# Blaizzy/mlx-audio

Hardware: NVIDIA H100
Metric: audio-sec/sec Kokoro-82M TTS (128-phoneme utterance, 9.75 s) (higher is better)
Workload: dtype bf16x2

## Files before the change

### include/b200audio.h

```cpp
#ifndef B200AUDIO_H
#define B200AUDIO_H

#include <stdint.h>

#ifdef __cplusplus
extern "C" {
#endif

#define B2A_OK 0
#define B2A_E_INVALID (-1)
#define B2A_E_CUDA (-2)
#define B2A_E_UNSUPPORTED (-3)

enum {
  B2A_ACT_NONE = 0,
  B2A_ACT_LRELU = 1,
  B2A_ACT_SNAKE = 2,
  B2A_ACT_ELU = 3,
  B2A_ACT_GELU = 4,
  B2A_ACT_GELU_TANH = 5,
  B2A_ACT_TANH = 6,
  B2A_ACT_SIGMOID = 7,
  B2A_ACT_SILU = 8,
  B2A_ACT_CLIP1 = 9
};

const char* b2a_last_error(void);
int32_t b2a_version(void);
int32_t b2a_device_sm_count(void);

typedef struct {
  const float* x; int64_t x_bs; int64_t x_ld;
  int32_t B, L, Cin;
  const float* w; const float* bias;
  float* y; int64_t y_bs; int64_t y_ld;
  int32_t Lout, Cout;
  int32_t K, stride, dilation, pad_left, groups, pad_mode;
  const float* pre_scale; const float* pre_shift;
  int32_t pre_act; float pre_p0; const float* pre_a; const float* pre_b;
  int32_t post_act; float post_p0;
  const float* post_cscale; int64_t post_cscale_bs;
  const float* res; int64_t res_bs; int64_t res_ld; int32_t res_div;
  float out_scale; int32_t accumulate;
  void* emit_hi; void* emit_lo; int64_t emit_ld;
  int32_t emit_act; float emit_p0; const float* emit_a; const float* emit_b;
} b2a_conv1d_t;

int32_t b2a_conv1d_cl(const b2a_conv1d_t* p, void* stream);
int32_t b2a_convtr1d_cl(const b2a_conv1d_t* p, void* stream);

enum {
  B2A_CONV_PATH_LINEAR_ROWS = 1,
  B2A_CONV_PATH_NARROW = 2,
  B2A_CONV_PATH_DENSE = 3,
  B2A_CONV_PATH_DW_TILED4 = 4,
  B2A_CONV_PATH_DW_TILED = 5,
  B2A_CONV_PATH_DW = 6,
  B2A_CONV_PATH_CONVTR_DENSE = 7,
  B2A_CONV_PATH_CONVTR_DW = 8
};
int32_t b2a_conv1d_cl_last_path(int32_t* out4);

int32_t b2a_kokoro_source_conv(const float* x, int32_t B, int32_t L, const float* w, const float* bias, float* y, int32_t Lout,
                               int32_t Cout, int32_t K, int32_t stride, int32_t pad_left, void* stream);

int32_t b2a_prep_bf16(const float* x, int64_t x_bs, int64_t x_ld, int32_t B, int32_t L, int32_t C, int32_t cpad,
                      const float* scale, const float* shift, int32_t act, float p0, const float* a, const float* b,
                      void* hi, void* lo, int32_t f16, void* stream);
int32_t b2a_conv1d_tc(const void* a_hi, const void* a_lo, int32_t f16, int32_t B, int32_t L, int32_t cin_pad, const void* w_bf16,
                      const void* w_lo,
                      int32_t taps, const int32_t* shifts_host, int32_t Cout, int32_t Lout, const float* bias,
                      int32_t post_act, float post_p0, const float* cscale, int64_t cscale_bs, const float* res,
                      int64_t res_bs, int64_t res_ld, int32_t res_div, float out_scale, int32_t accumulate, float* y,
                      int64_t y_bs, int64_t y_ld, int32_t up_stride, int32_t up_crop, void* emit_hi, void* emit_lo,
                      int64_t emit_ld, void* attn_ws, int32_t attn_heads, float attn_scale, void* stream);

typedef struct {
  int32_t T, layers, heads, hidden, inter, planes;
  const void* w[4];
  const float* bias[4];
  const float* ln_w[2];
  const float* ln_b[2];
  float eps, scale;
  float* h; void* h_hi; void* h_lo;
} b2a_albert_t;
int64_t b2a_albert_ws_bytes(int32_t T, int32_t heads, int32_t hidden, int32_t inter);
int32_t b2a_albert_encoder(const b2a_albert_t* a, void* ws, uint32_t* err, int64_t* timeline, void* stream);

int32_t b2a_conv1d_tc_debug(void* dbg8);

int32_t b2a_conv1d_tc_last_config(int32_t* out5);

int32_t b2a_copy2d(const float* src, int64_t src_ld, float* dst, int64_t dst_ld, int64_t rows, int32_t cols, void* stream);
int32_t b2a_gather_rows(const float* src, int64_t src_ld, const int64_t* idx, float* dst, int64_t dst_ld,
                        int64_t rows, int32_t cols, int64_t n_src_rows, const float* add, int64_t add_ld, int64_t add_period,
                        void* stream);
int32_t b2a_durations_to_index(const float* dur_f, const int64_t* dur_i, int32_t T, float speed, int64_t* pred_dur_out,
                               int64_t* idx_out, int64_t max_frames, int64_t* total_dev, void* stream);

int64_t b2a_adain_ws_bytes(int32_t B, int32_t L, int32_t C);
int32_t b2a_adain_coeffs(const float* x, int64_t x_bs, int64_t x_ld, int32_t B, int32_t L, int32_t C,
                         const float* gb, float eps, float* scale, float* shift, void* ws, void* stream);
int32_t b2a_channel_stats(const float* x, int64_t x_bs, int64_t x_ld, int32_t B, int32_t L, int32_t C, int64_t* const* dst,
                          const int64_t* dst_bs, int32_t n_dst, void* stream);
int32_t b2a_coeffs_from_stats(const int64_t* stats, int32_t B, int32_t L, int32_t C, const float* gb, float eps, float* scale, float* shift,
                              void* stream);
int32_t b2a_layernorm(const float* x, int64_t x_ld, const float* res, int64_t res_ld, float* y, int64_t y_ld,
                      int64_t rows, int32_t C, const float* w, const float* b, const float* ada, float eps,
                      int32_t rms, int32_t post_act, float post_p0, void* emit_hi, void* emit_lo, int64_t emit_ld, void* stream);

typedef struct {
  const float* q; const float* k; const float* v; float* o;
  int64_t q_bs, q_ld, k_bs, k_ld, v_bs, v_ld, o_bs, o_ld;
  int32_t B, Tq, Tk, H, Hkv, D;
  float scale; int32_t causal, q_offset, window;
  const int32_t* k_len;
  void* emit_hi; void* emit_lo; int64_t emit_ld;
  int32_t operands_ready;
} b2a_attn_t;
int32_t b2a_attention(const b2a_attn_t* p, void* stream);
int64_t b2a_attention_tc_ws_bytes(int32_t B, int32_t H, int32_t Tq, int32_t Tk);
int32_t b2a_attention_tc(const b2a_attn_t* p, void* ws, void* stream);
int32_t b2a_rope(float* x, int64_t x_bs, int64_t x_ld, int32_t B, int32_t T, int32_t H, int32_t D,
                 int32_t offset, float base, int32_t traditional, void* stream);

int32_t b2a_lstm_bidir(const float* xproj, const float* wh, float* out, int64_t out_ld, int32_t B, int32_t T, int32_t H, void* stream);

int32_t b2a_stft(const float* x, int64_t x_bs, int32_t B, int64_t n, const float* window, int32_t n_fft, int32_t hop,
                 int32_t pad_mode, int64_t frames, float* out_re, float* out_im, void* stream);
int32_t b2a_whisper_logmel(const float* x, int64_t x_bs, int32_t B, int64_t n, int64_t padding, const float* window,
                           const float* filters, int32_t n_mels, int64_t frames, float* out, float* gmax, void* stream);
int32_t b2a_istft(const float* re, const float* im, int32_t B, int32_t n_fft, int32_t T, int32_t hop, const float* window,
                  int32_t norm_sq, int32_t clamp_mode, int64_t trim, int64_t out_len, float* out, float* ws, void* stream);

int32_t b2a_resample_poly(const float* x, int64_t x_bs, int32_t B, int64_t n_in, const double* h, int32_t n_h, int32_t up,
                          int32_t down, int64_t n_pre_pad, int64_t n_pre_remove, float* out, int64_t n_out, void* stream);

int32_t b2a_kokoro_source(const float* f0, int32_t B, int32_t n_frames, int32_t n_down, const float* noise, const float* lin_w,
                          const float* lin_b, float* har, float* src_ws, double* ph_ws, void* stream);
int32_t b2a_kokoro_istft_head(const float* x, int64_t x_bs, int64_t x_ld, int32_t B, int32_t T, float* audio, void* stream);

#define B2A_CONVF_MAX_PROBLEMS 4
typedef struct {
  const float* x; const float* x1; const float* x2; int64_t x_bs, x_ld; float in_scale;
  int32_t B, L, Cin;
  int32_t pre_mode; const float* pre_scale; const float* pre_shift; const int64_t* pre_stats; const float* pre_gb; int64_t pre_gb_bs; float pre_eps;
  int32_t pre_act; float pre_p0; const float* pre_a; const float* pre_b;
  const void* w_hi; const void* w_lo; int32_t cin_pad, taps, N; int32_t shifts[32];
  int32_t Lout; const float* bias; int32_t post_act; float post_p0; const float* cscale; int64_t cscale_bs;
  const float* res; int64_t res_bs, res_ld; int32_t res_div; float out_scale; int32_t accumulate;
  float* y; int64_t y_bs, y_ld;
  int32_t up_stride, up_crop;
  int64_t* stats_out;
} b2a_convf_t;
int32_t b2a_conv1d_fused_debug(void* stamps );
int32_t b2a_conv1d_fused(const b2a_convf_t* problems, int32_t n_problems, int32_t planes, int32_t f16, void* ws, int64_t ws_bytes, void* stream);
int32_t b2a_conv1d_fused_fits(int32_t span, int32_t N, int32_t C, int32_t wplanes, int32_t planes);
int32_t b2a_conv1d_fused_last_config(int32_t* out10);

int32_t b2a_randn(float* out, int64_t n, uint64_t seed, uint64_t offset, void* stream);
int32_t b2a_randn_dev(float* out, int64_t n, uint64_t* state, void* stream);

int32_t b2a_whisper_greedy_step(const float* logits, int64_t logits_bs, const int64_t* tokens, int64_t tokens_bs,
                                int32_t B, int32_t cur_len, int32_t sample_begin, int32_t V, const float* suppress_mask,
                                const float* blank_mask, int32_t eot, int32_t no_timestamps, int32_t timestamp_begin,
                                int32_t max_initial_ts, int32_t without_timestamps, int64_t* next_out,
                                float* sum_logprobs, int32_t* not_done, float temperature, const float* u, void* stream);

int32_t b2a_sample_token(const float* logits, int64_t logits_bs, int32_t B, int32_t V, const float* suppress_mask,
                         uint8_t* seen, int64_t seen_bs, int32_t mark_seen, float repetition_penalty, float temperature,
                         int32_t top_k, float top_p, float min_p, const float* u, int64_t* out, int64_t out_stride,
                         float* filtered_out, uint8_t* finished, int32_t eos, void* stream);

int32_t b2a_gemv_bf16(const float* x, int64_t x_ld, int32_t M, int32_t K, const void* w_bf16, int64_t w_ld, int32_t N,
                      const float* bias, const float* norm_w, float norm_eps, int32_t mode, const float* res, int64_t res_ld,
                      float* y, int64_t y_ld, const void* prefetch, int64_t prefetch_bytes, void* stream);
int32_t b2a_qknorm_rope_cache(const float* qkv, int64_t qkv_bs, int64_t qkv_ss, int32_t B, int32_t S, int32_t Hq, int32_t Hkv,
                              int32_t D, const float* q_norm_w, const float* k_norm_w, float eps, const int32_t* pos3,
                              const int32_t* base_dev, int32_t base_host, int32_t sec_h, int32_t sec_w, float theta,
                              float* q_out, int64_t qo_bs, int64_t qo_ss, float* k_cache, float* v_cache, int64_t c_bs,
                              int64_t c_ss, int32_t smax, const int32_t* pos_shift, const int32_t* base_rows, const int32_t* slot,
                              void* stream);
int32_t b2a_attn_decode(const float* q, int64_t q_bs, int64_t q_ss, const float* k_cache, const float* v_cache, int64_t c_bs,
                        int64_t c_ss, float* out, int64_t o_bs, int64_t o_ss, int32_t B, int32_t S, int32_t Hq, int32_t Hkv,
                        int32_t D, float scale, const int32_t* base_dev, int32_t base_host, const int32_t* kv_start,
                        int32_t max_k, const int32_t* base_rows, const int32_t* slot, void* stream);
int32_t b2a_attn_prefill(const float* q, int64_t q_bs, int64_t q_ss, const float* k_cache, const float* v_cache, int64_t c_bs,
                         int64_t c_ss, float* out, int64_t o_bs, int64_t o_ss, int32_t B, int32_t S, int32_t Hq, int32_t Hkv,
                         int32_t D, float scale, const int32_t* base_dev, int32_t base_host, const int32_t* kv_start,
                         int32_t max_k, const int32_t* base_rows, const int32_t* slot, void* stream);
int32_t b2a_swiglu(const float* x, int64_t x_ld, int64_t rows, int32_t I, int32_t interleaved, float* y, int64_t y_ld, void* stream);
int32_t b2a_embed_sum(const int64_t* codes, int64_t codes_bs, int32_t B, int32_t G, int32_t dim, const float* const* tables_dev,
                      const int32_t* bins_dev, const float* text, int64_t text_bs, int64_t text_ss, int32_t n_text,
                      const float* pad, const int32_t* step_dev, int32_t step_sub, float* out, int64_t out_bs,
                      int32_t* err_flag_dev, int32_t* tidx, const uint8_t* finished, void* stream);
int32_t b2a_incr_i32(int32_t* p, int32_t v, void* stream);
int32_t b2a_slot_advance(int32_t* lengths, int32_t* frames, uint8_t* finished, const int32_t* cap, const int64_t* codes, int32_t G,
                         int64_t* out, int64_t out_bs, const float* u_tab, int64_t u_bs, float* u, int32_t B, void* stream);

int32_t b2a_rvq_decode(const int64_t* codes, int64_t codes_bs, int64_t codes_qs, int32_t B, int32_t nq, int64_t T,
                       const float* codebooks, int32_t bins, int32_t dim, float* out, int64_t out_ld, int32_t* err_flag_dev, void* stream);
int32_t b2a_rvq_encode(const float* x, int64_t x_ld, int64_t rows, int32_t dim, const float* codebooks, const double* c2, int32_t bins,
                       int32_t nq, int32_t mode, int64_t* codes, int64_t codes_row_stride, int64_t codes_level_stride, void* stream);
int32_t b2a_snac_from_codes(const int64_t* const* codes_host_ptrs, const int32_t* strides_host, int32_t n_levels,
                            const float* const* emb_host_ptrs, const float* const* w_host_ptrs, const float* const* bias_host_ptrs,
                            int32_t B, int64_t T, int32_t bins, int32_t cd, int32_t dim, float* out, int32_t* err_flag_dev, void* stream);

typedef struct {
  const float* w_in; const float* b_in;
  const float* cbn; const double* c2;
  const float* cb;
  const float* w_out; const float* b_out;
  int32_t cd; int32_t lat_off;
} b2a_dac_level_t;
int64_t b2a_dac_rvq_encode_smem_bytes(int32_t dim);
int32_t b2a_dac_rvq_encode(const float* z, int64_t z_ld, int32_t B, int64_t T, int32_t dim, const b2a_dac_level_t* levels_dev, int32_t n_levels,
                           int32_t bins, int32_t latent_channels, int64_t* codes, float* latents, float* z_q, double* loss_part, void* stream);
int32_t b2a_dac_from_codes(const int64_t* codes, int64_t codes_bs, int64_t codes_qs, int32_t B, int32_t n_levels, int64_t T,
                           const b2a_dac_level_t* levels_dev, int32_t bins, int32_t latent_channels, int32_t dim, float* out, float* z_p,
                           int32_t* err_flag_dev, void* stream);

int32_t b2a_aa_snakebeta(const float* x, int64_t x_bs, int64_t x_ld, int32_t B, int32_t L, int32_t C, const float* alpha, const float* inv_beta,
                         const float* f_up, const float* f_down, int32_t ratio, int32_t taps, float* y, int64_t y_bs, int64_t y_ld, void* hi,
                         void* lo, int32_t cpad, void* stream);

#define B2A_ROWOP_COPY 0
#define B2A_ROWOP_ADD 1
#define B2A_ROWOPS_MAX 32
typedef struct {
  const float* src; int64_t src_bs, src_ld;
  float* dst; int64_t dst_bs, dst_ld;
  int32_t B, rows, C, op;
} b2a_rowop_t;
int32_t b2a_stream_rows(const b2a_rowop_t* ops, int32_t n, void* stream);

int32_t b2a_conv1d_stream(const b2a_conv1d_t* p, float* hist, int64_t hist_bs, int32_t H, const int32_t* step_dev, int32_t fresh,
                          void* stream);
int32_t b2a_convtr1d_stream(const b2a_conv1d_t* p, float* tail, int64_t tail_bs, void* stream);
int32_t b2a_ring_rope_kv(float* qkv, int64_t qkv_bs, int64_t qkv_ld, int32_t B, int32_t T, int32_t H, int32_t D, float base,
                         float* k_ring, float* v_ring, int64_t ring_bs, int32_t cap, const int32_t* pos_dev, void* stream);
int32_t b2a_ring_attn(const float* q, int64_t q_bs, int64_t q_ld, const float* k_ring, const float* v_ring, int64_t ring_bs, int32_t cap,
                      float* out, int64_t o_bs, int64_t o_ld, int32_t B, int32_t T, int32_t H, int32_t D, float scale, int32_t window,
                      const int32_t* pos_dev, void* stream);
int32_t b2a_stream_advance(int32_t* ctr, int32_t dpos, void* stream);

int32_t b2a_spk_logmel(const float* x, int64_t x_bs, int32_t B, int64_t n, const float* window, const float* filters, int32_t n_mels,
                       int64_t frames, float* out, void* stream);
int32_t b2a_spk_reflect_pad(const float* x, int64_t x_bs, int64_t x_ld, int32_t B, int32_t T, int32_t C, int32_t pad, float* out_f32,
                            void* hi, void* lo, int32_t cpad, void* stream);
int64_t b2a_spk_res2net_smem_bytes(int32_t C, int32_t scale, int32_t K, int32_t pad, int32_t tile);
int32_t b2a_spk_res2net(const float* y, int64_t y_bs, int64_t y_ld, float* z, int64_t z_bs, int64_t z_ld, const float* w, const float* bias,
                        int32_t B, int32_t T, int32_t C, int32_t scale, int32_t K, int32_t dilation, int32_t tile, void* stream);
int32_t b2a_spk_channel_stats(const float* x, int64_t x_bs, int64_t x_ld, int32_t B, int32_t T, int32_t C, int32_t with_std, float eps,
                              float* out, int64_t o_bs, void* stream);
int32_t b2a_spk_se_gate(const float* mean, int64_t m_bs, int32_t B, int32_t C, int32_t S, const float* w1, const float* b1, const float* w2,
                        const float* b2, float* gate, void* stream);
int32_t b2a_spk_se_apply(const float* y, int64_t y_bs, int64_t y_ld, const float* gate, const float* res, int64_t r_bs, int64_t r_ld,
                         float* out, int64_t o_bs, int64_t o_ld, int32_t B, int32_t T, int32_t C, void* stream);
int32_t b2a_spk_gemv(const float* x, int64_t x_bs, int32_t B, int32_t K, const float* w, int64_t w_ld, int32_t N, const float* bias,
                     int32_t act, float* y, int64_t y_bs, void* stream);
int32_t b2a_spk_asp_act(float* h, int64_t h_bs, int64_t h_ld, const float* cb, int32_t B, int32_t T, int32_t A, void* stream);
int32_t b2a_spk_asp_pool(const float* logits, int64_t l_bs, int64_t l_ld, const float* x, int64_t x_bs, int64_t x_ld, int32_t B, int32_t T,
                         int32_t C, float eps, float* pooled, int64_t p_bs, void* stream);

int32_t b2a_vocos_dwnorm(const float* x, int64_t x_bs, int64_t x_ld, int32_t B, int32_t L, int32_t C, const float* dw_w, const float* dw_b,
                         int32_t K, const float* w, const float* b, const float* ada, int64_t ada_bs, float eps, float* y, int64_t y_bs,
                         int64_t y_ld, void* hi, void* lo, void* stream);
int32_t b2a_vocos_istft_head(const float* h, int64_t h_bs, int64_t h_ld, int32_t B, int32_t T, int32_t n_fft, int32_t hop, const float* window,
                             float* out, int64_t out_bs, void* stream);
int32_t b2a_vocos_logmel(const float* x, int64_t x_bs, int32_t B, int64_t n, const float* window, const float* filters, int32_t n_mels,
                         int64_t frames, float* out, void* stream);

int32_t b2a_encodec_lstm(const float* xproj, const float* wh, const float* skip, float* out, int32_t R, int32_t T, int32_t H, uint32_t* err,
                         void* stream);
int32_t b2a_encodec_pad(const float* x, int64_t x_bs, int64_t x_ld, int32_t B, int32_t T, int32_t C, int32_t pad_left, int32_t pad_right,
                        int32_t reflect, const float* scale, const float* shift, int32_t elu, const float* res, int64_t res_bs, int64_t res_ld,
                        float* y, int64_t y_bs, int64_t y_ld, void* stream);
int64_t b2a_encodec_gn_ws_bytes(int32_t B);
int32_t b2a_encodec_gn_coeffs(const float* x, int64_t x_bs, int64_t x_ld, int32_t B, int32_t T, int32_t C, const float* gamma,
                              const float* beta, float eps, float* scale, float* shift, void* ws, void* stream);
int32_t b2a_encodec_normalize(const float* x, int64_t x_bs, int64_t x_ld, int32_t R, int32_t L, int32_t C, const uint8_t* mask,
                              int64_t mask_bs, float* y, float* scale, void* stream);
int32_t b2a_encodec_ola(const float* frames, int32_t N, int32_t B, int32_t L, int32_t C, const float* scale, int32_t stride, int32_t Tout,
                        float* out, void* stream);

int32_t b2a_lm_sample_mlx(const float* logits, int64_t logits_bs, int32_t B, int32_t V, float temperature, double top_p, const float* u,
                          int64_t u_bs, const int32_t* step_dev, int64_t* out, int64_t* hist, int64_t hist_bs, uint8_t* finished,
                          int32_t stop0, int32_t stop1, void* stream);
int32_t b2a_soprano_upsample(const float* x, int64_t x_bs, int64_t x_ld, int32_t B, int32_t L, int32_t H, int32_t up, float* y, int64_t y_bs,
                             int64_t y_ld, void* hi, void* lo, int32_t cpad, void* stream);
int32_t b2a_soprano_store_rows(const float* src, int64_t src_bs, int32_t B, int32_t H, float* dst, int64_t dst_bs, int64_t dst_ld,
                               const int32_t* idx_dev, int32_t add, int32_t cap, void* stream);

#ifdef __cplusplus
}
#endif
#endif
```

### mlx_audio_b200/_lib.py

```python
from __future__ import annotations

import ctypes as C
import os

_HERE = os.path.dirname(os.path.abspath(__file__))
LIB_PATH = os.path.join(_HERE, "libb200audio.so")

c_f = C.c_void_p
i32, i64, f32 = C.c_int32, C.c_int64, C.c_float


class Conv1dParams(C.Structure):
    _fields_ = [
        ("x", C.c_void_p), ("x_bs", i64), ("x_ld", i64),
        ("B", i32), ("L", i32), ("Cin", i32),
        ("w", C.c_void_p), ("bias", C.c_void_p),
        ("y", C.c_void_p), ("y_bs", i64), ("y_ld", i64),
        ("Lout", i32), ("Cout", i32),
        ("K", i32), ("stride", i32), ("dilation", i32), ("pad_left", i32), ("groups", i32), ("pad_mode", i32),
        ("pre_scale", C.c_void_p), ("pre_shift", C.c_void_p),
        ("pre_act", i32), ("pre_p0", f32), ("pre_a", C.c_void_p), ("pre_b", C.c_void_p),
        ("post_act", i32), ("post_p0", f32),
        ("post_cscale", C.c_void_p), ("post_cscale_bs", i64),
        ("res", C.c_void_p), ("res_bs", i64), ("res_ld", i64), ("res_div", i32),
        ("out_scale", f32), ("accumulate", i32),
        ("emit_hi", C.c_void_p), ("emit_lo", C.c_void_p), ("emit_ld", i64),
        ("emit_act", i32), ("emit_p0", f32), ("emit_a", C.c_void_p), ("emit_b", C.c_void_p),
    ]


class AttnParams(C.Structure):
    _fields_ = [
        ("q", C.c_void_p), ("k", C.c_void_p), ("v", C.c_void_p), ("o", C.c_void_p),
        ("q_bs", i64), ("q_ld", i64), ("k_bs", i64), ("k_ld", i64), ("v_bs", i64), ("v_ld", i64), ("o_bs", i64), ("o_ld", i64),
        ("B", i32), ("Tq", i32), ("Tk", i32), ("H", i32), ("Hkv", i32), ("D", i32),
        ("scale", f32), ("causal", i32), ("q_offset", i32), ("window", i32),
        ("k_len", C.c_void_p),
        ("emit_hi", C.c_void_p), ("emit_lo", C.c_void_p), ("emit_ld", i64), ("operands_ready", i32),
    ]


class ConvFParams(C.Structure):
    _fields_ = [
        ("x", C.c_void_p), ("x1", C.c_void_p), ("x2", C.c_void_p), ("x_bs", i64), ("x_ld", i64), ("in_scale", f32),
        ("B", i32), ("L", i32), ("Cin", i32),
        ("pre_mode", i32), ("pre_scale", C.c_void_p), ("pre_shift", C.c_void_p), ("pre_stats", C.c_void_p), ("pre_gb", C.c_void_p),
        ("pre_gb_bs", i64), ("pre_eps", f32),
        ("pre_act", i32), ("pre_p0", f32), ("pre_a", C.c_void_p), ("pre_b", C.c_void_p),
        ("w_hi", C.c_void_p), ("w_lo", C.c_void_p), ("cin_pad", i32), ("taps", i32), ("N", i32), ("shifts", i32 * 32),
        ("Lout", i32), ("bias", C.c_void_p), ("post_act", i32), ("post_p0", f32), ("cscale", C.c_void_p), ("cscale_bs", i64),
        ("res", C.c_void_p), ("res_bs", i64), ("res_ld", i64), ("res_div", i32), ("out_scale", f32), ("accumulate", i32),
        ("y", C.c_void_p), ("y_bs", i64), ("y_ld", i64),
        ("up_stride", i32), ("up_crop", i32),
        ("stats_out", C.c_void_p),
    ]


class AlbertParams(C.Structure):
    _fields_ = [("T", i32), ("layers", i32), ("heads", i32), ("hidden", i32), ("inter", i32), ("planes", i32),
                ("w", C.c_void_p * 4), ("bias", C.c_void_p * 4), ("ln_w", C.c_void_p * 2), ("ln_b", C.c_void_p * 2),
                ("eps", f32), ("scale", f32), ("h", C.c_void_p), ("h_hi", C.c_void_p), ("h_lo", C.c_void_p)]


class RowOp(C.Structure):
    _fields_ = [("src", C.c_void_p), ("src_bs", i64), ("src_ld", i64), ("dst", C.c_void_p), ("dst_bs", i64), ("dst_ld", i64),
                ("B", i32), ("rows", i32), ("C", i32), ("op", i32)]


class DacLevel(C.Structure):
    _fields_ = [("w_in", C.c_void_p), ("b_in", C.c_void_p), ("cbn", C.c_void_p), ("c2", C.c_void_p), ("cb", C.c_void_p),
                ("w_out", C.c_void_p), ("b_out", C.c_void_p), ("cd", i32), ("lat_off", i32)]


ROWOPS_MAX = 32


PROTOTYPES = {
    "b2a_last_error": (C.c_char_p, []),
    "b2a_version": (i32, []),
    "b2a_device_sm_count": (i32, []),
    "b2a_conv1d_cl": (i32, [C.POINTER(Conv1dParams), C.c_void_p]),
    "b2a_convtr1d_cl": (i32, [C.POINTER(Conv1dParams), C.c_void_p]),
    "b2a_conv1d_cl_last_path": (i32, [C.POINTER(i32)]),
    "b2a_kokoro_source_conv": (i32, [c_f, i32, i32, c_f, c_f, c_f, i32, i32, i32, i32, i32, C.c_void_p]),
    "b2a_prep_bf16": (i32, [c_f, i64, i64, i32, i32, i32, i32, c_f, c_f, i32, f32, c_f, c_f, c_f, c_f, i32, C.c_void_p]),
    "b2a_conv1d_tc": (i32, [c_f, c_f, i32, i32, i32, i32, c_f, c_f, i32, C.POINTER(i32), i32, i32, c_f, i32, f32, c_f, i64, c_f, i64, i64, i32, f32, i32,
                            c_f, i64, i64, i32, i32, c_f, c_f, i64, c_f, i32, f32, C.c_void_p]),
    "b2a_conv1d_tc_debug": (i32, [c_f]),
    "b2a_conv1d_tc_last_config": (i32, [C.POINTER(i32)]),
    "b2a_conv1d_fused_debug": (i32, [c_f]),
    "b2a_conv1d_fused_last_config": (i32, [C.POINTER(i32)]),
    "b2a_conv1d_fused": (i32, [C.POINTER(ConvFParams), i32, i32, i32, c_f, i64, C.c_void_p]),
    "b2a_conv1d_fused_fits": (i32, [i32, i32, i32, i32, i32]),
    "b2a_copy2d": (i32, [c_f, i64, c_f, i64, i64, i32, C.c_void_p]),
    "b2a_gather_rows": (i32, [c_f, i64, c_f, c_f, i64, i64, i32, i64, c_f, i64, i64, C.c_void_p]),
    "b2a_durations_to_index": (i32, [c_f, c_f, i32, f32, c_f, c_f, i64, c_f, C.c_void_p]),
    "b2a_adain_ws_bytes": (i64, [i32, i32, i32]),
    "b2a_adain_coeffs": (i32, [c_f, i64, i64, i32, i32, i32, c_f, f32, c_f, c_f, c_f, C.c_void_p]),
    "b2a_channel_stats": (i32, [c_f, i64, i64, i32, i32, i32, C.POINTER(C.c_void_p), C.POINTER(i64), i32, C.c_void_p]),
    "b2a_coeffs_from_stats": (i32, [c_f, i32, i32, i32, c_f, f32, c_f, c_f, C.c_void_p]),
    "b2a_layernorm": (i32, [c_f, i64, c_f, i64, c_f, i64, i64, i32, c_f, c_f, c_f, f32, i32, i32, f32, c_f, c_f, i64, C.c_void_p]),
    "b2a_attention": (i32, [C.POINTER(AttnParams), C.c_void_p]),
    "b2a_attention_tc_ws_bytes": (i64, [i32, i32, i32, i32]),
    "b2a_attention_tc": (i32, [C.POINTER(AttnParams), C.c_void_p, C.c_void_p]),
    "b2a_albert_ws_bytes": (i64, [i32, i32, i32, i32]),
    "b2a_albert_encoder": (i32, [C.POINTER(AlbertParams), C.c_void_p, C.c_void_p, C.c_void_p, C.c_void_p]),
    "b2a_rope": (i32, [c_f, i64, i64, i32, i32, i32, i32, i32, f32, i32, C.c_void_p]),
    "b2a_lstm_bidir": (i32, [c_f, c_f, c_f, i64, i32, i32, i32, C.c_void_p]),
    "b2a_stft": (i32, [c_f, i64, i32, i64, c_f, i32, i32, i32, i64, c_f, c_f, C.c_void_p]),
    "b2a_whisper_logmel": (i32, [c_f, i64, i32, i64, i64, c_f, c_f, i32, i64, c_f, c_f, C.c_void_p]),
    "b2a_istft": (i32, [c_f, c_f, i32, i32, i32, i32, c_f, i32, i32, i64, i64, c_f, c_f, C.c_void_p]),
    "b2a_resample_poly": (i32, [c_f, i64, i32, i64, c_f, i32, i32, i32, i64, i64, c_f, i64, C.c_void_p]),
    "b2a_kokoro_source": (i32, [c_f, i32, i32, i32, c_f, c_f, c_f, c_f, c_f, c_f, C.c_void_p]),
    "b2a_kokoro_istft_head": (i32, [c_f, i64, i64, i32, i32, c_f, C.c_void_p]),
    "b2a_randn": (i32, [c_f, i64, C.c_uint64, C.c_uint64, C.c_void_p]),
    "b2a_randn_dev": (i32, [c_f, i64, c_f, C.c_void_p]),
    "b2a_whisper_greedy_step": (i32, [c_f, i64, c_f, i64, i32, i32, i32, i32, c_f, c_f, i32, i32, i32, i32, i32, c_f, c_f, c_f, f32, c_f, C.c_void_p]),
    "b2a_sample_token": (i32, [c_f, i64, i32, i32, c_f, c_f, i64, i32, f32, f32, i32, f32, f32, c_f, c_f, i64, c_f, c_f, i32, C.c_void_p]),
    "b2a_gemv_bf16": (i32, [c_f, i64, i32, i32, c_f, i64, i32, c_f, c_f, f32, i32, c_f, i64, c_f, i64, c_f, i64, C.c_void_p]),
    "b2a_qknorm_rope_cache": (i32, [c_f, i64, i64, i32, i32, i32, i32, i32, c_f, c_f, f32, c_f, c_f, i32, i32, i32, f32, c_f, i64, i64,
                                    c_f, c_f, i64, i64, i32, c_f, c_f, c_f, C.c_void_p]),
    "b2a_attn_decode": (i32, [c_f, i64, i64, c_f, c_f, i64, i64, c_f, i64, i64, i32, i32, i32, i32, i32, f32, c_f, i32, c_f, i32, c_f, c_f,
                              C.c_void_p]),
    "b2a_attn_prefill": (i32, [c_f, i64, i64, c_f, c_f, i64, i64, c_f, i64, i64, i32, i32, i32, i32, i32, f32, c_f, i32, c_f, i32, c_f, c_f,
                               C.c_void_p]),
    "b2a_swiglu": (i32, [c_f, i64, i64, i32, i32, c_f, i64, C.c_void_p]),
    "b2a_embed_sum": (i32, [c_f, i64, i32, i32, i32, c_f, c_f, c_f, i64, i64, i32, c_f, c_f, i32, c_f, i64, c_f, c_f, c_f, C.c_void_p]),
    "b2a_incr_i32": (i32, [c_f, i32, C.c_void_p]),
    "b2a_slot_advance": (i32, [c_f, c_f, c_f, c_f, c_f, i32, c_f, i64, c_f, i64, c_f, i32, C.c_void_p]),
    "b2a_rvq_decode": (i32, [c_f, i64, i64, i32, i32, i64, c_f, i32, i32, c_f, i64, c_f, C.c_void_p]),
    "b2a_rvq_encode": (i32, [c_f, i64, i64, i32, c_f, c_f, i32, i32, i32, c_f, i64, i64, C.c_void_p]),
    "b2a_snac_from_codes": (i32, [C.POINTER(C.c_void_p), C.POINTER(i32), i32, C.POINTER(C.c_void_p), C.POINTER(C.c_void_p),
                                  C.POINTER(C.c_void_p), i32, i64, i32, i32, i32, c_f, c_f, C.c_void_p]),
    "b2a_dac_rvq_encode_smem_bytes": (i64, [i32]),
    "b2a_dac_rvq_encode": (i32, [c_f, i64, i32, i64, i32, c_f, i32, i32, i32, c_f, c_f, c_f, c_f, C.c_void_p]),
    "b2a_dac_from_codes": (i32, [c_f, i64, i64, i32, i32, i64, c_f, i32, i32, i32, c_f, c_f, c_f, C.c_void_p]),
    "b2a_aa_snakebeta": (i32, [c_f, i64, i64, i32, i32, i32, c_f, c_f, c_f, c_f, i32, i32, c_f, i64, i64, c_f, c_f, i32, C.c_void_p]),
    "b2a_stream_rows": (i32, [C.POINTER(RowOp), i32, C.c_void_p]),
    "b2a_conv1d_stream": (i32, [C.POINTER(Conv1dParams), c_f, i64, i32, c_f, i32, C.c_void_p]),
    "b2a_convtr1d_stream": (i32, [C.POINTER(Conv1dParams), c_f, i64, C.c_void_p]),
    "b2a_ring_rope_kv": (i32, [c_f, i64, i64, i32, i32, i32, i32, f32, c_f, c_f, i64, i32, c_f, C.c_void_p]),
    "b2a_ring_attn": (i32, [c_f, i64, i64, c_f, c_f, i64, i32, c_f, i64, i64, i32, i32, i32, i32, f32, i32, c_f, C.c_void_p]),
    "b2a_stream_advance": (i32, [c_f, i32, C.c_void_p]),
    "b2a_spk_logmel": (i32, [c_f, i64, i32, i64, c_f, c_f, i32, i64, c_f, C.c_void_p]),
    "b2a_spk_reflect_pad": (i32, [c_f, i64, i64, i32, i32, i32, i32, c_f, c_f, c_f, i32, C.c_void_p]),
    "b2a_spk_res2net_smem_bytes": (i64, [i32, i32, i32, i32, i32]),
    "b2a_spk_res2net": (i32, [c_f, i64, i64, c_f, i64, i64, c_f, c_f, i32, i32, i32, i32, i32, i32, i32, C.c_void_p]),
    "b2a_spk_channel_stats": (i32, [c_f, i64, i64, i32, i32, i32, i32, f32, c_f, i64, C.c_void_p]),
    "b2a_spk_se_gate": (i32, [c_f, i64, i32, i32, i32, c_f, c_f, c_f, c_f, c_f, C.c_void_p]),
    "b2a_spk_se_apply": (i32, [c_f, i64, i64, c_f, c_f, i64, i64, c_f, i64, i64, i32, i32, i32, C.c_void_p]),
    "b2a_spk_gemv": (i32, [c_f, i64, i32, i32, c_f, i64, i32, c_f, i32, c_f, i64, C.c_void_p]),
    "b2a_spk_asp_act": (i32, [c_f, i64, i64, c_f, i32, i32, i32, C.c_void_p]),
    "b2a_spk_asp_pool": (i32, [c_f, i64, i64, c_f, i64, i64, i32, i32, i32, f32, c_f, i64, C.c_void_p]),
    "b2a_vocos_dwnorm": (i32, [c_f, i64, i64, i32, i32, i32, c_f, c_f, i32, c_f, c_f, c_f, i64, f32, c_f, i64, i64, c_f, c_f, C.c_void_p]),
    "b2a_vocos_istft_head": (i32, [c_f, i64, i64, i32, i32, i32, i32, c_f, c_f, i64, C.c_void_p]),
    "b2a_vocos_logmel": (i32, [c_f, i64, i32, i64, c_f, c_f, i32, i64, c_f, C.c_void_p]),
    "b2a_encodec_lstm": (i32, [c_f, c_f, c_f, c_f, i32, i32, i32, c_f, C.c_void_p]),
    "b2a_encodec_pad": (i32, [c_f, i64, i64, i32, i32, i32, i32, i32, i32, c_f, c_f, i32, c_f, i64, i64, c_f, i64, i64, C.c_void_p]),
    "b2a_encodec_gn_ws_bytes": (i64, [i32]),
    "b2a_encodec_gn_coeffs": (i32, [c_f, i64, i64, i32, i32, i32, c_f, c_f, f32, c_f, c_f, c_f, C.c_void_p]),
    "b2a_encodec_normalize": (i32, [c_f, i64, i64, i32, i32, i32, c_f, i64, c_f, c_f, C.c_void_p]),
    "b2a_encodec_ola": (i32, [c_f, i32, i32, i32, i32, c_f, i32, i32, c_f, C.c_void_p]),
    "b2a_lm_sample_mlx": (i32, [c_f, i64, i32, i32, f32, C.c_double, c_f, i64, c_f, c_f, c_f, i64, c_f, i32, i32, C.c_void_p]),
    "b2a_soprano_upsample": (i32, [c_f, i64, i64, i32, i32, i32, i32, c_f, i64, i64, c_f, c_f, i32, C.c_void_p]),
    "b2a_soprano_store_rows": (i32, [c_f, i64, i32, i32, c_f, i64, i64, c_f, i32, i32, C.c_void_p]),
}

E_INVALID, E_CUDA, E_UNSUPPORTED = -1, -2, -3


def load() -> C.CDLL:
    if not os.path.exists(LIB_PATH):
        raise ImportError(
            f"{LIB_PATH} is missing: build it with `python -m mlx_audio_b200.build` "
            "(there is no CPU or PyTorch fallback for the hot path)")
    lib = C.CDLL(LIB_PATH)
    for name, (res, args) in PROTOTYPES.items():
        fn = getattr(lib, name)
        fn.restype = res
        fn.argtypes = args
    return lib


_LIB = None


def lib() -> C.CDLL:
    global _LIB
    if _LIB is None:
        _LIB = load()
    return _LIB


def check(rc: int) -> None:
    if rc == 0:
        return
    msg = lib().b2a_last_error().decode("utf-8", "replace")
    if rc == E_INVALID:
        raise ValueError(msg)
    if rc == E_UNSUPPORTED:
        raise NotImplementedError(msg)
    raise RuntimeError(msg)
```

### mlx_audio_b200/csrc/albert.cu

```cuda
#include "common.cuh"
#include "tc_common.cuh"
#include "tc_epilogue.cuh"
#include "attn_tc_tile.cuh"
#include "layernorm_row.cuh"

using namespace tc;

namespace {

constexpr int THREADS = 288;
constexpr int SLOTS = 6;
constexpr int SLOT_BYTES = 32768;
constexpr int PLANE = 64 * 128;
constexpr int OFF_Q = SLOTS * SLOT_BYTES;
constexpr int OFF_BAR = OFF_Q + 2 * PLANE;
constexpr int SMEM_BYTES = OFF_BAR + (2 * SLOTS + 2) * 8 + 16 + 1024;
constexpr int STAGES = 7;
constexpr long long TIMEOUT_NS = 10000000000LL;

struct AlbertMaps {
  CUtensorMap a_hi[4], a_lo[4], w[4];
  CUtensorMap qh, ql, kh, kl, vh, vl;
};

struct AlbertParams {
  int T, layers, planes, mb, H, hs, inter, nkt;
  int N[4], K[4];
  const float* bias[4];
  const float *ln_w[2], *ln_b[2]; float eps;
  float qmul;
  float *h, *t, *u;
  __nv_bfloat16 *hp_hi, *hp_lo, *ap_hi, *ap_lo, *fp_hi, *fp_lo;
  __nv_bfloat16 *cp_hi, *cp_lo;
  AttnOperands attn;
  unsigned* bar; unsigned* err;
  long long* tl;
};

__device__ __forceinline__ int gemm_of_stage(int s) { return s == 0 ? 0 : s == 2 ? 1 : s == 4 ? 2 : s == 5 ? 3 : -1; }

__device__ __forceinline__ long long globaltimer() {
  long long t;
  asm volatile("mov.u64 %0, %globaltimer;" : "=l"(t));
  return t;
}

__device__ bool grid_wait(const AlbertParams& p, unsigned target) {
  long long t0 = 0;
  for (int it = 0;; it++) {
    unsigned v;
    asm volatile("ld.acquire.gpu.global.u32 %0, [%1];" : "=r"(v) : "l"(p.bar) : "memory");
    if ((int)(v - target) >= 0) return true;
    if ((it & 63) == 63) {
      if (*(volatile unsigned*)p.err) return false;
      const long long now = globaltimer();
      if (!t0) t0 = now;
      else if (now - t0 > TIMEOUT_NS) { atomicExch(p.err, 1u); return false; }
    }
    __nanosleep(64);
  }
}

__device__ __forceinline__ void grid_arrive(unsigned* bar) {
  asm volatile("red.release.gpu.global.add.u32 [%0], 1;" ::"l"(bar) : "memory");
}

__device__ __forceinline__ void fence_proxy_async_global() { asm volatile("fence.proxy.async.global;" ::: "memory"); }

template <bool TL>
__global__ void __launch_bounds__(THREADS, 1) albert_kernel(const __grid_constant__ AlbertMaps maps, const AlbertParams p) {
  extern __shared__ __align__(1024) uint8_t smem_raw[];
  uint8_t* smem = (uint8_t*)(((uintptr_t)smem_raw + 1023) & ~(uintptr_t)1023);
  uint64_t* full = (uint64_t*)(smem + OFF_BAR);
  uint64_t* empty = full + SLOTS;
  uint64_t* q_full = empty + SLOTS;
  uint64_t* q_empty = q_full + 1;
  const int warp = threadIdx.x >> 5, lane = threadIdx.x & 31;
  const int bid = blockIdx.x, grid = gridDim.x;
  const int total = p.layers * STAGES;

  if (warp == 8 && lane == 0) {
    for (int g = 0; g < 4; g++) {
      asm volatile("prefetch.tensormap [%0];" ::"l"(&maps.a_hi[g]) : "memory");
      asm volatile("prefetch.tensormap [%0];" ::"l"(&maps.w[g]) : "memory");
    }
    for (int s = 0; s < SLOTS; s++) { mbar_init(full + s, 1); mbar_init(empty + s, 2); }
    mbar_init(q_full, 1); mbar_init(q_empty, 2);
    asm volatile("fence.mbarrier_init.release.cluster;" ::: "memory");
    asm volatile("fence.proxy.async.shared::cta;" ::: "memory");
  }
  __syncthreads();

  if (warp == 8) {
    if (lane != 0) return;
    uint32_t g = 0, qn = 0;
    for (int k = 0; k < total; k++) {
      const int stage = k % STAGES, gi = gemm_of_stage(stage);
      if (stage == 1) {
        const int units = p.H * p.mb;
        if (bid >= units) continue;
        grid_wait(p, (unsigned)k * grid);
        fence_proxy_async_global();
        for (int u = bid; u < units; u += grid) {
          const int head = u / p.mb, q0 = (u % p.mb) * 64;
          mbar_wait(q_empty, (qn & 1) ^ 1);
          mbar_expect_tx(q_full, 2 * PLANE);
          tma_load_3d(smem + OFF_Q, &maps.qh, q_full, 0, q0, head);
          tma_load_3d(smem + OFF_Q + PLANE, &maps.ql, q_full, 0, q0, head);
          qn++;
          for (int t = 0; t < p.nkt; t++, g++) {
            const int s = g % SLOTS;
            uint8_t* st = smem + (size_t)s * SLOT_BYTES;
            mbar_wait(empty + s, ((g / SLOTS) & 1) ^ 1);
            mbar_expect_tx(full + s, 4 * PLANE);
            tma_load_3d(st, &maps.kh, full + s, 0, t * 64, head);
            tma_load_3d(st + PLANE, &maps.kl, full + s, 0, t * 64, head);
            tma_load_3d(st + 2 * PLANE, &maps.vh, full + s, t * 64, 0, head);
            tma_load_3d(st + 3 * PLANE, &maps.vl, full + s, t * 64, 0, head);
          }
        }
        continue;
      }
      if (gi < 0) continue;
      const int units = p.mb * (p.N[gi] / 64), kc = p.K[gi] / 64;
      const uint32_t bytes = (uint32_t)(PLANE * p.planes + PLANE);
      bool waited = k == 0;
      for (int u = bid; u < units; u += grid) {
        const int m0 = (u % p.mb) * 64, n0 = (u / p.mb) * 64;
        int pre = 0;
        if (!waited) {
          pre = kc < SLOTS ? kc : SLOTS;
          for (int c = 0; c < pre; c++) {
            const uint32_t gc = g + c;
            const int s = gc % SLOTS;
            mbar_wait(empty + s, ((gc / SLOTS) & 1) ^ 1);
            mbar_expect_tx(full + s, bytes);
            tma_load_2d(smem + (size_t)s * SLOT_BYTES + 2 * PLANE, &maps.w[gi], full + s, c * 64, n0);
          }
          grid_wait(p, (unsigned)k * grid);
          fence_proxy_async_global();
          waited = true;
          for (int c = 0; c < pre; c++) {
            const int s = (g + c) % SLOTS;
            uint8_t* st = smem + (size_t)s * SLOT_BYTES;
            tma_load_2d(st, &maps.a_hi[gi], full + s, c * 64, m0);
            if (p.planes == 2) tma_load_2d(st + PLANE, &maps.a_lo[gi], full + s, c * 64, m0);
          }
        }
        for (int c = pre; c < kc; c++) {
          const uint32_t gc = g + c;
          const int s = gc % SLOTS;
          uint8_t* st = smem + (size_t)s * SLOT_BYTES;
          mbar_wait(empty + s, ((gc / SLOTS) & 1) ^ 1);
          mbar_expect_tx(full + s, bytes);
          tma_load_2d(st + 2 * PLANE, &maps.w[gi], full + s, c * 64, n0);
          tma_load_2d(st, &maps.a_hi[gi], full + s, c * 64, m0);
          if (p.planes == 2) tma_load_2d(st + PLANE, &maps.a_lo[gi], full + s, c * 64, m0);
        }
        g += kc;
      }
    }
    return;
  }

  const int ct = threadIdx.x, wg = warp >> 2, w4 = warp & 3;
  const uint32_t sb = smem_u32(smem);
  uint32_t g = 0, qn = 0;
  for (int k = 0; k < total; k++) {
    const int stage = k % STAGES, gi = gemm_of_stage(stage);
    if (k > 0) {
      if (ct == 0) grid_wait(p, (unsigned)k * grid);
      bar_sync(1, 256);
    }
    if constexpr (TL) { if (ct == 0) p.tl[((int64_t)k * grid + bid) * 2] = globaltimer(); }
    if (gi >= 0) {
      const int units = p.mb * (p.N[gi] / 64), kc = p.K[gi] / 64, N = p.N[gi];
      const float* bias = p.bias[gi];
      for (int u = bid; u < units; u += grid) {
        const int m0 = (u % p.mb) * 64, n0 = (u / p.mb) * 64;
        float acc[16];
        int prev = -1;
        for (int c = 0; c < kc; c++, g++) {
          const int s = g % SLOTS;
          mbar_wait(full + s, (g / SLOTS) & 1);
          const uint32_t st = sb + s * SLOT_BYTES;
          const uint64_t ad = gmma_desc_sw128(st), wd = gmma_desc_sw128(st + 2 * PLANE + wg * 32 * 128);
          wgmma_fence();
          wgmma_chunk<1, false>(acc, ad, wd, c != 0);
          if (p.planes == 2) wgmma_chunk<1, false>(acc, gmma_desc_sw128(st + PLANE), wd, 1u);
          wgmma_commit();
          wgmma_wait<1>();
          wgmma_fence_regs<16>(acc);
          if (prev >= 0 && (ct & 127) == 0) mbar_arrive(empty + prev);
          prev = s;
        }
        wgmma_wait<0>();
        wgmma_fence_regs<16>(acc);
        if ((ct & 127) == 0) mbar_arrive(empty + prev);
#pragma unroll
        for (int j = 0; j < 4; j++) {
          const int n = n0 + wg * 32 + 8 * j + 2 * (lane & 3);
          const float b0 = __ldg(bias + n), b1 = __ldg(bias + n + 1);
          EmitCol e0{}, e1{};
          if (gi == 0) { e0 = emit_col_attn(p.attn, 0, p.T, p.hs, p.qmul, n); e1 = emit_col_attn(p.attn, 0, p.T, p.hs, p.qmul, n + 1); }
#pragma unroll
          for (int hh = 0; hh < 2; hh++) {
            const int row = m0 + 16 * w4 + (lane >> 2) + 8 * hh;
            const float a0 = acc[4 * j + 2 * hh], a1 = acc[4 * j + 2 * hh + 1];
            if (row >= p.T) {
              if (gi == 0 && e0.step == 1 && row < p.attn.tkp) { e0.hi[row] = 0; e0.lo[row] = 0; e1.hi[row] = 0; e1.lo[row] = 0; }
              continue;
            }
            const int64_t o = (int64_t)row * N + n;
            if (gi == 0) {
              emit_store(e0, row, epilogue_value(a0, b0, 0, 0.f, 1.f, 0.f));
              emit_store(e1, row, epilogue_value(a1, b1, 0, 0.f, 1.f, 0.f));
            } else if (gi == 2) {
              const float y0 = epilogue_value(a0, b0, B2A_ACT_GELU, 0.f, 1.f, 0.f), y1 = epilogue_value(a1, b1, B2A_ACT_GELU, 0.f, 1.f, 0.f);
              __nv_bfloat162 h2, l2;
              split16(y0, h2.x, l2.x);
              split16(y1, h2.y, l2.y);
              *reinterpret_cast<__nv_bfloat162*>(p.fp_hi + o) = h2;
              if (p.planes == 2) *reinterpret_cast<__nv_bfloat162*>(p.fp_lo + o) = l2;
            } else {
              const float* res = gi == 1 ? p.h : p.t;
              float* out = gi == 1 ? p.t : p.u;
              const float2 r = *reinterpret_cast<const float2*>(res + o);
              *reinterpret_cast<float2*>(out + o) = make_float2(epilogue_value(a0, b0, 0, 0.f, 1.f, r.x), epilogue_value(a1, b1, 0, 0.f, 1.f, r.y));
            }
          }
        }
      }
    } else if (stage == 1) {
      const int units = p.H * p.mb;
      for (int u = bid; u < units; u += grid, qn++) {
        const int head = u / p.mb, q0 = (u % p.mb) * 64;
        float o[32], m[2] = {-INFINITY, -INFINITY}, l[2] = {0.f, 0.f};
#pragma unroll
        for (int j = 0; j < 32; j++) o[j] = 0.f;
        const int kmax[2] = {p.T - 1, p.T - 1}, kmin[2] = {0, 0};
        const uint64_t dqh = gmma_desc_sw128(sb + OFF_Q), dql = gmma_desc_sw128(sb + OFF_Q + PLANE);
        mbar_wait(q_full, qn & 1);
        for (int t = 0; t < p.nkt; t++, g++) {
          const int s = g % SLOTS;
          const uint32_t st = sb + s * SLOT_BYTES;
          mbar_wait(full + s, (g / SLOTS) & 1);
          if (wg == 0)
            attn_tc_tile(o, m, l, dqh, dql, gmma_desc_sw128(st), gmma_desc_sw128(st + PLANE), gmma_desc_sw128(st + 2 * PLANE),
                         gmma_desc_sw128(st + 3 * PLANE), t * 64, kmax, kmin, lane);
          if ((ct & 127) == 0) mbar_arrive(empty + s);
        }
        if ((ct & 127) == 0) mbar_arrive(q_empty);
        if (wg == 0) {
          float inv[2];
          attn_tc_row_inv(l, inv);
#pragma unroll
          for (int hh = 0; hh < 2; hh++) {
            const int q = q0 + w4 * 16 + (lane >> 2) + 8 * hh;
            if (q < p.T) {
              const int64_t e = (int64_t)q * p.hs + head * 64 + 2 * (lane & 3);
#pragma unroll
              for (int j = 0; j < 8; j++) {
                __nv_bfloat162 eh, el;
                split16(o[4 * j + 2 * hh] * inv[hh], eh.x, el.x);
                split16(o[4 * j + 2 * hh + 1] * inv[hh], eh.y, el.y);
                *reinterpret_cast<__nv_bfloat162*>(p.cp_hi + e + 8 * j) = eh;
                if (p.planes == 2) *reinterpret_cast<__nv_bfloat162*>(p.cp_lo + e + 8 * j) = el;
              }
            }
          }
        }
      }
    } else {
      const int which = stage == 3 ? 0 : 1;
      const float* x = which ? p.u : p.t;
      float* y = which ? p.h : p.t;
      __nv_bfloat16* eh = which ? p.hp_hi : p.ap_hi;
      __nv_bfloat16* el = p.planes == 2 ? (which ? p.hp_lo : p.ap_lo) : nullptr;
      for (int row = bid * 8 + warp; row < p.T; row += grid * 8) {
        const int64_t o = (int64_t)row * p.hs;
        layernorm_row_vec<8>(x + o, nullptr, y + o, p.hs, p.ln_w[which], p.ln_b[which], nullptr, p.eps, 0, 0, 0.f, eh + o,
                             el ? el + o : nullptr, lane);
      }
    }
    if constexpr (TL) { if (ct == 0) p.tl[((int64_t)k * grid + bid) * 2 + 1] = globaltimer(); }
    if (k + 1 < total) {
      fence_proxy_async_global();
      bar_sync(1, 256);
      if (ct == 0) { __threadfence(); grid_arrive(p.bar); }
    }
  }
}

typedef CUresult (*EncodeTiledFn)(CUtensorMap*, CUtensorMapDataType, cuuint32_t, void*, const cuuint64_t*, const cuuint64_t*,
                                  const cuuint32_t*, const cuuint32_t*, CUtensorMapInterleave, CUtensorMapSwizzle,
                                  CUtensorMapL2promotion, CUtensorMapFloatOOBfill);
EncodeTiledFn g_enc = nullptr;

int map16(CUtensorMap* m, const void* base, int rank, const uint64_t* dims, const uint64_t* strides_bytes, bool f16) {
  if (!g_enc) {
    void* fn = nullptr;
    cudaDriverEntryPointQueryResult qres;
    if (cudaGetDriverEntryPoint("cuTensorMapEncodeTiled", &fn, cudaEnableDefault, &qres) != cudaSuccess || !fn) return -1;
    g_enc = (EncodeTiledFn)fn;
  }
  cuuint64_t gd[3]; cuuint64_t gs[2]; cuuint32_t bx[3] = {64, 64, 1}; cuuint32_t es[3] = {1, 1, 1};
  for (int i = 0; i < rank; i++) gd[i] = dims[i];
  for (int i = 0; i < rank - 1; i++) gs[i] = strides_bytes[i];
  CUresult r = g_enc(m, f16 ? CU_TENSOR_MAP_DATA_TYPE_FLOAT16 : CU_TENSOR_MAP_DATA_TYPE_BFLOAT16, (cuuint32_t)rank, const_cast<void*>(base), gd,
                     gs, bx, es, CU_TENSOR_MAP_INTERLEAVE_NONE, CU_TENSOR_MAP_SWIZZLE_128B, CU_TENSOR_MAP_L2_PROMOTION_L2_256B,
                     CU_TENSOR_MAP_FLOAT_OOB_FILL_NONE);
  return r == CUDA_SUCCESS ? 0 : (int)r;
}

struct WsLayout { int64_t t, u, cp_hi, cp_lo, ap_hi, ap_lo, fp_hi, fp_lo, attn, total; };
WsLayout ws_layout(int64_t T, int64_t H, int64_t hs, int64_t inter) {
  auto up = [](int64_t x) { return (x + 255) / 256 * 256; };
  WsLayout w;
  int64_t o = 256;
  w.t = o; o += up(T * hs * 4);
  w.u = o; o += up(T * hs * 4);
  w.cp_hi = o; o += up(T * hs * 2);
  w.cp_lo = o; o += up(T * hs * 2);
  w.ap_hi = o; o += up(T * hs * 2);
  w.ap_lo = o; o += up(T * hs * 2);
  w.fp_hi = o; o += up(T * inter * 2);
  w.fp_lo = o; o += up(T * inter * 2);
  w.attn = o; o += b2a_attention_tc_ws_bytes(1, (int32_t)H, (int32_t)T, (int32_t)T);
  w.total = o;
  return w;
}

}

extern "C" int64_t b2a_albert_ws_bytes(int32_t T, int32_t heads, int32_t hidden, int32_t inter) {
  return ws_layout(T, heads, hidden, inter).total;
}

extern "C" int32_t b2a_albert_encoder(const b2a_albert_t* a, void* ws, uint32_t* err, int64_t* timeline, void* stream) {
  B2A_CHECK_ARG(a && ws && err && a->h && a->h_hi && (a->planes == 1 || (a->planes == 2 && a->h_lo)), "null pointer");
  for (int i = 0; i < 4; i++) B2A_CHECK_ARG(a->w[i] && a->bias[i], "null weight or bias");
  for (int i = 0; i < 2; i++) B2A_CHECK_ARG(a->ln_w[i] && a->ln_b[i], "null LayerNorm parameter");
  B2A_CHECK_ARG(a->T >= 64 && a->T <= 512 && a->layers > 0 && a->heads > 0 && a->hidden == 64 * a->heads && a->hidden <= 1024 &&
                a->inter % 64 == 0 && a->inter > 0, "shape: 64 <= T <= 512, hidden = 64 * heads <= 1024, inter a multiple of 64");
  const int T = a->T, H = a->heads, hs = a->hidden, inter = a->inter;
  uint8_t* base = (uint8_t*)ws;
  B2A_CHECK_ARG(((uintptr_t)base & 255) == 0, "workspace must be 256-byte aligned");
  const WsLayout L = ws_layout(T, H, hs, inter);
  cudaStream_t st = (cudaStream_t)stream;

  AlbertParams p{};
  p.T = T; p.layers = a->layers; p.planes = a->planes; p.mb = cdiv(T, 64); p.H = H; p.hs = hs; p.inter = inter; p.nkt = cdiv(T, 64);
  const int N[4] = {3 * hs, hs, inter, hs}, K[4] = {hs, hs, hs, inter};
  for (int i = 0; i < 4; i++) { p.N[i] = N[i]; p.K[i] = K[i]; p.bias[i] = a->bias[i]; }
  for (int i = 0; i < 2; i++) { p.ln_w[i] = a->ln_w[i]; p.ln_b[i] = a->ln_b[i]; }
  p.eps = a->eps;
  p.qmul = a->scale * 1.4426950408889634f;
  p.h = a->h; p.t = (float*)(base + L.t); p.u = (float*)(base + L.u);
  p.hp_hi = (__nv_bfloat16*)a->h_hi; p.hp_lo = (__nv_bfloat16*)a->h_lo;
  p.cp_hi = (__nv_bfloat16*)(base + L.cp_hi); p.cp_lo = (__nv_bfloat16*)(base + L.cp_lo);
  p.ap_hi = (__nv_bfloat16*)(base + L.ap_hi); p.ap_lo = (__nv_bfloat16*)(base + L.ap_lo);
  p.fp_hi = (__nv_bfloat16*)(base + L.fp_hi); p.fp_lo = (__nv_bfloat16*)(base + L.fp_lo);
  p.attn = attn_operands(base + L.attn, H, T, T);
  p.bar = (unsigned*)base; p.err = err;
  p.tl = (long long*)timeline;

  AlbertMaps m;
  const void* a_hi[4] = {p.hp_hi, p.cp_hi, p.ap_hi, p.fp_hi};
  const void* a_lo[4] = {p.hp_lo, p.cp_lo, p.ap_lo, p.fp_lo};
  int e = 0;
  for (int i = 0; i < 4 && !e; i++) {
    const uint64_t ad[2] = {(uint64_t)K[i], (uint64_t)T}, as[1] = {(uint64_t)K[i] * 2};
    const uint64_t wd[2] = {(uint64_t)K[i], (uint64_t)N[i]};
    e = map16(&m.a_hi[i], a_hi[i], 2, ad, as, false);
    if (!e) e = map16(&m.a_lo[i], a->planes == 2 ? a_lo[i] : a_hi[i], 2, ad, as, false);
    if (!e) e = map16(&m.w[i], a->w[i], 2, wd, as, false);
  }
  const uint64_t qd[3] = {64, (uint64_t)T, (uint64_t)H}, qs[2] = {128, (uint64_t)T * 128};
  const uint64_t vd[3] = {(uint64_t)p.attn.tkp, 64, (uint64_t)H}, vs[2] = {(uint64_t)p.attn.tkp * 2, (uint64_t)p.attn.tkp * 128};
  if (!e) e = map16(&m.qh, p.attn.qh, 3, qd, qs, true);
  if (!e) e = map16(&m.ql, p.attn.ql, 3, qd, qs, true);
  if (!e) e = map16(&m.kh, p.attn.kh, 3, qd, qs, true);
  if (!e) e = map16(&m.kl, p.attn.kl, 3, qd, qs, true);
  if (!e) e = map16(&m.vh, p.attn.vh, 3, vd, vs, true);
  if (!e) e = map16(&m.vl, p.attn.vl, 3, vd, vs, true);
  if (e) { b2a_set_error("b2a_albert_encoder: cuTensorMapEncodeTiled failed (%d)", e); return B2A_E_CUDA; }

  void (*kern)(const AlbertMaps, const AlbertParams) = timeline ? albert_kernel<true> : albert_kernel<false>;
  static bool attr[2] = {false, false};
  if (!attr[timeline ? 1 : 0]) {
    if (cudaFuncSetAttribute(kern, cudaFuncAttributeMaxDynamicSharedMemorySize, SMEM_BYTES) != cudaSuccess) {
      b2a_set_error("b2a_albert_encoder: cannot raise the dynamic shared-memory limit: %s", cudaGetErrorString(cudaGetLastError()));
      return B2A_E_CUDA;
    }
    attr[timeline ? 1 : 0] = true;
  }
  int dev = 0, nsm = 0, per_sm = 0;
  cudaGetDevice(&dev);
  cudaDeviceGetAttribute(&nsm, cudaDevAttrMultiProcessorCount, dev);
  if (cudaOccupancyMaxActiveBlocksPerMultiprocessor(&per_sm, kern, THREADS, SMEM_BYTES) != cudaSuccess || per_sm < 1 || nsm < 1) {
    b2a_set_error("b2a_albert_encoder: the kernel cannot be resident (%s)", cudaGetErrorString(cudaGetLastError()));
    return B2A_E_CUDA;
  }
  if (cudaMemsetAsync(p.bar, 0, 4, st) != cudaSuccess) { b2a_set_error("b2a_albert_encoder: %s", cudaGetErrorString(cudaGetLastError())); return B2A_E_CUDA; }
  cudaLaunchConfig_t cfg = {};
  cfg.gridDim = dim3(nsm); cfg.blockDim = dim3(THREADS); cfg.dynamicSmemBytes = SMEM_BYTES; cfg.stream = st;
  cudaLaunchAttribute at[1];
  at[0].id = cudaLaunchAttributeCooperative;
  at[0].val.cooperative = 1;
  cfg.attrs = at; cfg.numAttrs = 1;
  if (cudaLaunchKernelEx(&cfg, kern, m, p) != cudaSuccess) {
    b2a_set_error("b2a_albert_encoder: %s", cudaGetErrorString(cudaGetLastError()));
    return B2A_E_CUDA;
  }
  return B2A_OK;
}
```

### mlx_audio_b200/ops.py

```python
from __future__ import annotations

import ctypes as C
import math
import contextlib
import os
from dataclasses import dataclass
from typing import Optional

import torch

from . import _lib
from ._lib import AttnParams, Conv1dParams, ConvFParams

ACT = {"none": 0, "lrelu": 1, "snake": 2, "elu": 3, "gelu": 4, "gelu_tanh": 5, "tanh": 6, "sigmoid": 7,
       "silu": 8, "clip1": 9}

LAUNCHES = [0]


PROFILE = None
PROFILE_TAGS = None
TAG = [None]
PROFILE_EXTERNAL = False


def _call(kind, fn, n_launches, *args):
    if PROFILE is not None:
        a = torch.cuda.Event(enable_timing=True, external=PROFILE_EXTERNAL)
        b = torch.cuda.Event(enable_timing=True, external=PROFILE_EXTERNAL)
        a.record()
        rc = fn(*args)
        b.record()
        PROFILE.setdefault(kind, []).append((a, b))
        if PROFILE_TAGS is not None:
            PROFILE_TAGS.setdefault(kind, []).append(TAG[0])
        TAG[0] = None
    else:
        rc = fn(*args)
    _lib.check(rc)
    LAUNCHES[0] += n_launches


_SIDE_POOL = {}
_SIDE_BUSY = set()


def fork(device, n: int = 1):
    device = torch.device(device)
    cur = torch.cuda.current_stream(device)
    pool = _SIDE_POOL.setdefault(device, [])
    out = []
    for s in pool:
        if len(out) == n:
            break
        if s not in _SIDE_BUSY and s != cur:
            out.append(s)
    while len(out) < n:
        s = torch.cuda.Stream(device=device)
        pool.append(s)
        out.append(s)
    for s in out:
        _SIDE_BUSY.add(s)
        s.wait_stream(cur)
    return out


def join(device, streams) -> None:
    cur = torch.cuda.current_stream(torch.device(device))
    for s in streams:
        cur.wait_stream(s)
        _SIDE_BUSY.discard(s)


def _stream() -> int:
    return torch.cuda.current_stream().cuda_stream


def _p(t: Optional[torch.Tensor]):
    return None if t is None else t.data_ptr()


def _chk3(x: torch.Tensor, name: str):
    if x.dtype != torch.float32 or not x.is_cuda or x.dim() != 3 or x.stride(2) != 1:
        raise ValueError(f"{name}: expected a CUDA float32 [B, L, C] tensor with unit channel stride, got "
                         f"{tuple(x.shape)} {x.dtype} {x.device} strides {x.stride()}")


@dataclass
class Pre:
    scale: Optional[torch.Tensor] = None
    shift: Optional[torch.Tensor] = None
    act: int = 0
    p0: float = 0.0
    a: Optional[torch.Tensor] = None
    b: Optional[torch.Tensor] = None


@dataclass
class ConvW:
    w: torch.Tensor
    bias: Optional[torch.Tensor]
    K: int
    cin: int
    cout: int
    groups: int = 1
    w_tc: Optional[torch.Tensor] = None
    cin_pad: int = 0
    f16: bool = False
    w_tc_lo: Optional[torch.Tensor] = None


TC_MODE = [os.environ.get("B2A_TC", "x2")]
ATTN_MODE = [os.environ.get("B2A_ATTN", "tc")]
TC_MIN_K = 32


def _tc_eligible(cw: "ConvW", L: int, stride: int, transpose: bool, pad_mode: int, dilation: int = 1) -> bool:
    if TC_MODE[0] == "off" or cw.w_tc is None or pad_mode != 0 or cw.cout % 32 != 0 or L < 32:
        return False
    if transpose:
        return dilation == 1 and cw.K % stride == 0 and cw.cin * (cw.K // stride) >= TC_MIN_K
    return stride == 1 and cw.cin * cw.K >= TC_MIN_K


def _tc_transposed_weights(cw: "ConvW", stride: int):
    cache = cw.__dict__.setdefault("_w_tc_tr", {})
    if stride not in cache:
        J = cw.K // stride
        w = cw.w.reshape(J, stride, cw.cin, cw.cout).permute(0, 1, 3, 2).reshape(J, stride * cw.cout, cw.cin)
        wt = torch.zeros(J, stride * cw.cout, cw.cin_pad, device=cw.w.device, dtype=cw.w_tc.dtype)
        wt[:, :, :cw.cin] = w.to(cw.w_tc.dtype)
        wl = None
        if cw.w_tc_lo is not None:
            wl = torch.zeros_like(wt)
            wl[:, :, :cw.cin] = (w - wt[:, :, :cw.cin].float()).to(wt.dtype)
        cache[stride] = (wt.contiguous(), None if wl is None else wl.contiguous())
    return cache[stride]


@dataclass
class Planes:
    hi: torch.Tensor
    lo: Optional[torch.Tensor]
    C: int

    @property
    def shape(self):
        return (self.hi.shape[0], self.hi.shape[1], self.C)


def pack_conv(w_mlx: torch.Tensor, bias=None, groups=1, device="cuda") -> ConvW:
    cout, k, cin_g = w_mlx.shape
    if groups == 1:
        w = w_mlx.permute(1, 2, 0).contiguous()
        cin = cin_g
    else:
        if not (cin_g == 1 and groups == cout):
            raise NotImplementedError("only dense or depthwise convolutions are on the hot path")
        w = w_mlx[:, :, 0].t().contiguous()
        cin = cout
    cwo = ConvW(w.to(device=device, dtype=torch.float32), None if bias is None else bias.to(device=device, dtype=torch.float32).contiguous(),
                k, cin, cout, groups)
    if groups == 1 and cout % 32 == 0 and torch.device(device).type == "cuda":
        for dt in (torch.bfloat16, torch.float16):
            wb = w_mlx.float().to(dt)
            if torch.equal(wb.float(), w_mlx.float()):
                cpad = -(-cin // 64) * 64
                wt = torch.zeros(k, cout, cpad, dtype=dt)
                wt[:, :, :cin] = wb.permute(1, 0, 2)
                cwo.w_tc, cwo.cin_pad, cwo.f16 = wt.to(device).contiguous(), cpad, dt == torch.float16
                break
        else:
            cpad = -(-cin // 64) * 64
            w32 = w_mlx.float().permute(1, 0, 2)
            hi = w32.to(torch.bfloat16)
            lo = (w32 - hi.float()).to(torch.bfloat16)
            wt, wl = torch.zeros(k, cout, cpad, dtype=torch.bfloat16), torch.zeros(k, cout, cpad, dtype=torch.bfloat16)
            wt[:, :, :cin], wl[:, :, :cin] = hi, lo
            cwo.w_tc, cwo.w_tc_lo, cwo.cin_pad = wt.to(device).contiguous(), wl.to(device).contiguous(), cpad
    return cwo


def pack_linear(w: torch.Tensor, bias=None, device="cuda") -> ConvW:
    return pack_conv(w[:, None, :], bias, 1, device)


def conv1d(x: torch.Tensor, cw: ConvW, *, stride=1, dilation=1, pad_left=0, lout=None, pad_mode=0,
           pre: Optional[Pre] = None, post_act=0, post_p0=0.0, cscale=None, res=None, res_div=1,
           out_scale=1.0, out=None, accumulate=False, transpose=False, emit: Optional[Pre] = None):
    if isinstance(x, Planes):
        B, L, cin = x.shape
        if (cin != cw.cin or pre is not None or not _tc_eligible(cw, L, stride, transpose, pad_mode, dilation) or x.hi.shape[2] != cw.cin_pad
                or x.hi.dtype != (torch.float16 if cw.f16 else torch.bfloat16)):
            raise ValueError("conv1d: a Planes operand needs a tensor-core-eligible layer with matching channels, dtype and no prologue")
        if lout is None:
            lout = (L + 2 * pad_left - dilation * (cw.K - 1) - 1) // stride + 1
        return _conv1d_tc(x, cw, dilation, pad_left, lout, None, post_act, post_p0, cscale, res, res_div, out_scale, out, accumulate,
                          up_stride=stride if transpose else 0)
    _chk3(x, "conv1d x")
    B, L, cin = x.shape
    if cin != cw.cin:
        raise ValueError(f"conv1d: input has {cin} channels, weight expects {cw.cin}")
    if lout is None:
        if transpose:
            lout = (L - 1) * stride + cw.K - 2 * pad_left
        else:
            lout = (L + 2 * pad_left - dilation * (cw.K - 1) - 1) // stride + 1
    small_gemm = cw.K == 1 and B * L <= 256 and _tc_eligible(cw, L, stride, transpose, pad_mode, dilation)
    if FUSED_DISPATCH[0] and emit is None and not small_gemm and fused_eligible(x, cw, stride, dilation, transpose, pad_mode, out, res):
        y = conv_fused(FusedProblem(x, cw, stride=stride, dilation=dilation, pad_left=pad_left, lout=lout, pre=pre, post_act=post_act,
                                    post_p0=post_p0, cscale=cscale, res=res, res_div=res_div, out_scale=out_scale, out=out,
                                    accumulate=accumulate, transpose=transpose))[0]
        return y
    if _tc_eligible(cw, L, stride, transpose, pad_mode, dilation):
        return _conv1d_tc(x, cw, dilation, pad_left, lout, pre, post_act, post_p0, cscale, res, res_div, out_scale, out, accumulate,
                          up_stride=stride if transpose else 0)
    planes = None
    if emit is not None:
        if not emit_eligible(cw, x, lout, stride, dilation, transpose) or res is not None or cscale is not None or accumulate or post_act or out is not None:
            raise ValueError("conv1d: emit= needs a stride-1 depthwise layer with Cout % 64 == 0 and no epilogue extras (see ops.emit_eligible)")
        planes = Planes(torch.empty(B, lout, cw.cout, device=x.device, dtype=torch.bfloat16),
                        torch.empty(B, lout, cw.cout, device=x.device, dtype=torch.bfloat16) if TC_MODE[0] == "x2" else None, cw.cout)
    elif out is None:
        out = torch.empty(B, lout, cw.cout, device=x.device, dtype=torch.float32)
    else:
        _chk3(out, "conv1d out")
        if out.shape != (B, lout, cw.cout):
            raise ValueError(f"conv1d: out has shape {tuple(out.shape)}, expected {(B, lout, cw.cout)}")
    p = Conv1dParams()
    p.x, p.x_bs, p.x_ld = x.data_ptr(), x.stride(0), x.stride(1)
    p.B, p.L, p.Cin = B, L, cin
    p.w, p.bias = cw.w.data_ptr(), _p(cw.bias)
    if planes is None:
        p.y, p.y_bs, p.y_ld = out.data_ptr(), out.stride(0), out.stride(1)
    else:
        p.emit_hi, p.emit_lo, p.emit_ld = planes.hi.data_ptr(), _p(planes.lo), cw.cout
        p.emit_act, p.emit_p0, p.emit_a, p.emit_b = emit.act, emit.p0, _p(emit.a), _p(emit.b)
    p.Lout, p.Cout = lout, cw.cout
    p.K, p.stride, p.dilation, p.pad_left, p.groups, p.pad_mode = cw.K, stride, dilation, pad_left, cw.groups, pad_mode
    if pre is not None:
        p.pre_scale, p.pre_shift = _p(pre.scale), _p(pre.shift)
        p.pre_act, p.pre_p0, p.pre_a, p.pre_b = pre.act, pre.p0, _p(pre.a), _p(pre.b)
    p.post_act, p.post_p0 = post_act, post_p0
    if cscale is not None:
        p.post_cscale = cscale.data_ptr()
        p.post_cscale_bs = cscale.stride(0) if cscale.dim() == 2 else 0
    if res is not None:
        _chk3(res, "conv1d res")
        p.res, p.res_bs, p.res_ld = res.data_ptr(), (res.stride(0) if res.shape[0] == B else 0), res.stride(1)
    p.res_div = res_div
    p.out_scale, p.accumulate = out_scale, int(accumulate)
    fn = _lib.lib().b2a_convtr1d_cl if transpose else _lib.lib().b2a_conv1d_cl
    if PROFILE_TAGS is not None:
        TAG[0] = f"cuda-core conv [{B}x{L}x{cw.cin}->{cw.cout} k{cw.K} s{stride} d{dilation} g{cw.groups}{' T' if transpose else ''}]"
    _call("conv" if cw.groups == 1 and cw.cin * cw.K >= 64 else "other", fn, 1, C.byref(p), _stream())
    if planes is not None:
        return planes
    return out


def emit_eligible(cw: "ConvW", x: torch.Tensor, lout: int, stride: int = 1, dilation: int = 1, transpose: bool = False) -> bool:
    return (TC_MODE[0] != "off" and not transpose and stride == 1 and cw.groups == cw.cin == cw.cout and cw.cout % 64 == 0 and cw.K <= 16
            and lout >= 128 and x.stride(1) % 4 == 0 and x.stride(0) % 4 == 0 and x.data_ptr() % 16 == 0
            and (128 + (cw.K - 1) * dilation) * 128 * 4 <= 160 * 1024)


def emit_tc_eligible(cw: "ConvW", L: int) -> bool:
    return cw.K == 1 and not cw.f16 and cw.cout % 64 == 0 and _tc_eligible(cw, L, 1, False, 0)


def prep_bf16(x: torch.Tensor, pre: Optional[Pre], cpad: int, planes: int = 2, f16: bool = False):
    _chk3(x, "prep_bf16 x")
    B, L, Cc = x.shape
    dt = torch.float16 if f16 else torch.bfloat16
    hi = torch.empty(B, L, cpad, device=x.device, dtype=dt)
    lo = torch.empty(B, L, cpad, device=x.device, dtype=dt) if planes == 2 else None
    pre = pre or Pre()
    _call("prep", _lib.lib().b2a_prep_bf16, 1, x.data_ptr(), x.stride(0), x.stride(1), B, L, Cc, cpad, _p(pre.scale), _p(pre.shift),
          pre.act, pre.p0, _p(pre.a), _p(pre.b), hi.data_ptr(), _p(lo), int(f16), _stream())
    return hi, lo


def _new_planes(B: int, L: int, C: int, device) -> Planes:
    return Planes(torch.empty(B, L, C, device=device, dtype=torch.bfloat16),
                  torch.empty(B, L, C, device=device, dtype=torch.bfloat16) if TC_MODE[0] == "x2" else None, C)


@dataclass
class AttnPlanes:
    ws: torch.Tensor
    B: int
    T: int
    H: int


def _conv1d_tc(x, cw, dilation, pad_left, lout, pre, post_act, post_p0, cscale, res, res_div, out_scale, out, accumulate,
               up_stride=0, emit: Optional[Planes] = None, attn: Optional[AttnPlanes] = None, attn_scale=0.0):
    if isinstance(x, Planes):
        B, L, _ = x.shape
        hi, lo = x.hi, x.lo
    else:
        B, L, _ = x.shape
        hi, lo = prep_bf16(x, pre, cw.cin_pad, 2 if TC_MODE[0] == "x2" else 1, cw.f16)
    if out is None:
        out = torch.empty(B, lout, cw.cout, device=hi.device, dtype=torch.float32)
    else:
        _chk3(out, "conv1d out")
        if out.shape != (B, lout, cw.cout):
            raise ValueError(f"conv1d: out has shape {tuple(out.shape)}, expected {(B, lout, cw.cout)}")
    if up_stride:
        taps, n_total = cw.K // up_stride, up_stride * cw.cout
        w_tc, w_lo = _tc_transposed_weights(cw, up_stride)
        shifts = (C.c_int32 * taps)(*[-j for j in range(taps)])
    else:
        taps, n_total, w_tc, w_lo = cw.K, cw.cout, cw.w_tc, cw.w_tc_lo
        shifts = (C.c_int32 * taps)(*[k * dilation - pad_left for k in range(taps)])
    cs, cs_bs = (None, 0) if cscale is None else (cscale.data_ptr(), cscale.stride(0) if cscale.dim() == 2 else 0)
    r, r_bs, r_ld = (None, 0, 0)
    if res is not None:
        _chk3(res, "conv1d res")
        r, r_bs, r_ld = res.data_ptr(), (res.stride(0) if res.shape[0] == B else 0), res.stride(1)
    _call("conv_tc", _lib.lib().b2a_conv1d_tc, 1, hi.data_ptr(), _p(lo), int(cw.f16), B, L, cw.cin_pad, w_tc.data_ptr(), _p(w_lo), taps, shifts, n_total, lout,
          _p(cw.bias), post_act, post_p0, cs, cs_bs, r, r_bs, r_ld, res_div, out_scale, int(accumulate), out.data_ptr(), out.stride(0),
          out.stride(1), up_stride, pad_left if up_stride else 0,
          None if emit is None else emit.hi.data_ptr(), None if emit is None else _p(emit.lo), 0 if emit is None else emit.hi.stride(1),
          None if attn is None else attn.ws.data_ptr(), 0 if attn is None else attn.H, float(attn_scale), _stream())
    return out


CL_PATHS = {1: "linear_rows", 2: "narrow", 3: "dense", 4: "dw_tiled4", 5: "dw_tiled", 6: "dw", 7: "convtr_dense", 8: "convtr_dw"}


def conv1d_cl_last_path() -> dict:
    out = (C.c_int32 * 4)()
    _lib.check(_lib.lib().b2a_conv1d_cl_last_path(out))
    return {"kernel": CL_PATHS.get(out[0]), "variant": (out[1], out[2], out[3])}


def conv1d_tc_last_config() -> dict:
    out = (C.c_int32 * 5)()
    _lib.check(_lib.lib().b2a_conv1d_tc_last_config(out))
    return {"BN": out[0], "grid": (out[1], out[2], out[3]), "stages": out[4]}


def conv1d_fused_last_config() -> dict:
    out = (C.c_int32 * 10)()
    _lib.check(_lib.lib().b2a_conv1d_fused_last_config(out))
    n = out[0]
    return {"grid": out[1], "BN": [out[2 + 2 * i] for i in range(n)], "ksplit": [out[3 + 2 * i] for i in range(n)]}


FUSED = [os.environ.get("B2A_FUSED", "1") != "0"]
FUSED_DISPATCH = [os.environ.get("B2A_FUSED_DISPATCH", "0") == "1"]


@contextlib.contextmanager
def fused_dispatch(on: bool = True):
    old = FUSED_DISPATCH[0]
    FUSED_DISPATCH[0] = bool(on) and FUSED[0]
    try:
        yield
    finally:
        FUSED_DISPATCH[0] = old
FUSED_WS_BYTES = 16 << 20
_FUSED_WS = {}


@dataclass
class PreStats:
    stats: torch.Tensor
    gb: Optional[torch.Tensor] = None
    eps: float = 1e-5
    act: int = 0
    p0: float = 0.0
    a: Optional[torch.Tensor] = None
    b: Optional[torch.Tensor] = None


STAT_BINS, STAT_BIN0, STAT_BIN_BITS = 4, -100, 40


def new_stats(B: int, Cc: int, device) -> torch.Tensor:
    return torch.zeros(B, Cc, 2, STAT_BINS, device=device, dtype=torch.int64)


def stats_value(stats: torch.Tensor) -> torch.Tensor:
    w = torch.tensor([2.0 ** (STAT_BIN0 + STAT_BIN_BITS * k) for k in range(STAT_BINS)], dtype=torch.float64, device=stats.device)
    t = torch.zeros(stats.shape[:-1], dtype=torch.float64, device=stats.device)
    for k in range(STAT_BINS - 1, -1, -1):
        t = t + stats[..., k].double() * w[k]
    return t


def _al16(t: Optional[torch.Tensor]) -> bool:
    return t is None or (t.data_ptr() % 16 == 0 and t.stride(1) % 4 == 0 and t.stride(0) % 4 == 0)


def fused_eligible(x, cw: "ConvW", stride: int = 1, dilation: int = 1, transpose: bool = False, pad_mode: int = 0, out=None, res=None) -> bool:
    if not FUSED[0] or TC_MODE[0] == "off" or cw.w_tc is None or pad_mode != 0 or cw.cout % 32 != 0 or cw.groups != 1 or isinstance(x, Planes):
        return False
    if x.dtype != torch.float32 or x.dim() != 3 or x.stride(2) != 1 or x.stride(1) % 4 or x.stride(0) % 4 or x.data_ptr() % 16:
        return False
    if x.stride(1) < -(-x.shape[2] // 4) * 4 or not _al16(out) or not _al16(res):
        return False
    if transpose:
        if not (dilation == 1 and cw.K % stride == 0 and cw.K // stride <= 32 and cw.cin * (cw.K // stride) >= TC_MIN_K):
            return False
        span, n_total = cw.K // stride - 1, stride * cw.cout
    else:
        if not (stride == 1 and cw.K <= 32 and cw.cin * cw.K >= TC_MIN_K):
            return False
        span, n_total = (cw.K - 1) * dilation, cw.cout
    return bool(_lib.lib().b2a_conv1d_fused_fits(span, n_total, cw.cout, 1 if cw.w_tc_lo is None else 2, 2 if TC_MODE[0] == "x2" else 1))


class FusedProblem:

    def __init__(self, x, cw: "ConvW", *, stride=1, dilation=1, pad_left=0, lout=None, pre=None, x_add=(), in_scale=1.0, post_act=0, post_p0=0.0,
                 cscale=None, res=None, res_div=1, out_scale=1.0, out=None, accumulate=False, transpose=False, stats_out=None):
        _chk3(x, "conv_fused x")
        B, L, cin = x.shape
        if cin != cw.cin:
            raise ValueError(f"conv_fused: input has {cin} channels, weight expects {cw.cin}")
        if lout is None:
            lout = (L - 1) * stride + cw.K - 2 * pad_left if transpose else (L + 2 * pad_left - dilation * (cw.K - 1) - 1) + 1
        if out is None:
            out = torch.empty(B, lout, cw.cout, device=x.device, dtype=torch.float32)
        else:
            _chk3(out, "conv_fused out")
            if out.shape != (B, lout, cw.cout):
                raise ValueError(f"conv_fused: out has shape {tuple(out.shape)}, expected {(B, lout, cw.cout)}")
        p = ConvFParams()
        p.x, p.x_bs, p.x_ld, p.in_scale = x.data_ptr(), x.stride(0), x.stride(1), float(in_scale)
        keep = [x, out, cw]
        for i, xa in enumerate(x_add):
            if xa.shape != x.shape or xa.stride() != x.stride() or xa.dtype != torch.float32:
                raise ValueError("conv_fused: x_add tensors must have x's shape and strides")
            setattr(p, "x1" if i == 0 else "x2", xa.data_ptr())
            keep.append(xa)
        p.B, p.L, p.Cin = B, L, cin
        if isinstance(pre, PreStats):
            if pre.stats.dtype != torch.int64 or tuple(pre.stats.shape) != (B, cin, 2, STAT_BINS) or not pre.stats.is_contiguous():
                raise ValueError("conv_fused: stats must be a contiguous int64 [B, Cin, 2, 4] tensor (ops.new_stats)")
            p.pre_mode, p.pre_stats, p.pre_eps = 2, pre.stats.data_ptr(), float(pre.eps)
            if pre.gb is not None:
                if pre.gb.shape[-1] != 2 * cin or pre.gb.stride(-1) != 1:
                    raise ValueError("conv_fused: gb must be [B, 2*Cin] rows (gamma | beta)")
                p.pre_gb, p.pre_gb_bs = pre.gb.data_ptr(), (pre.gb.stride(0) if pre.gb.dim() == 2 and pre.gb.shape[0] == B and B > 1 else 0)
            keep += [pre.stats, pre.gb]
        elif pre is not None and pre.scale is not None:
            p.pre_mode, p.pre_scale, p.pre_shift = 1, pre.scale.data_ptr(), pre.shift.data_ptr()
            keep += [pre.scale, pre.shift]
        if pre is not None:
            p.pre_act, p.pre_p0, p.pre_a, p.pre_b = pre.act, float(pre.p0), _p(pre.a), _p(pre.b)
            keep += [pre.a, pre.b]
        if transpose:
            taps, n_total = cw.K // stride, stride * cw.cout
            w_tc, w_lo = _tc_transposed_weights(cw, stride)
            shifts = [-j for j in range(taps)]
            p.up_stride, p.up_crop = stride, pad_left
        else:
            taps, n_total, w_tc, w_lo = cw.K, cw.cout, cw.w_tc, cw.w_tc_lo
            shifts = [k * dilation - pad_left for k in range(taps)]
        p.w_hi, p.w_lo, p.cin_pad, p.taps, p.N = w_tc.data_ptr(), _p(w_lo), cw.cin_pad, taps, n_total
        for i, sft in enumerate(shifts):
            p.shifts[i] = sft
        p.Lout, p.bias, p.post_act, p.post_p0 = lout, _p(cw.bias), post_act, float(post_p0)
        if cscale is not None:
            p.cscale, p.cscale_bs = cscale.data_ptr(), (cscale.stride(0) if cscale.dim() == 2 else 0)
            keep.append(cscale)
        if res is not None:
            _chk3(res, "conv_fused res")
            p.res, p.res_bs, p.res_ld = res.data_ptr(), (res.stride(0) if res.shape[0] == B else 0), res.stride(1)
            keep.append(res)
        p.res_div, p.out_scale, p.accumulate = res_div, float(out_scale), int(accumulate)
        p.y, p.y_bs, p.y_ld = out.data_ptr(), out.stride(0), out.stride(1)
        if stats_out is not None:
            if stats_out.dtype != torch.int64 or tuple(stats_out.shape) != (B, cw.cout, 2, STAT_BINS) or not stats_out.is_contiguous():
                raise ValueError("conv_fused: stats_out must be a contiguous int64 [B, Cout, 2, 4] tensor (ops.new_stats)")
            p.stats_out = stats_out.data_ptr()
            keep.append(stats_out)
        self.p, self.out, self.keep, self.f16 = p, out, keep, cw.f16


def conv_fused(problems) -> list:
    if isinstance(problems, FusedProblem):
        problems = [problems]
    n = len(problems)
    if not 1 <= n <= 4:
        raise ValueError("conv_fused: 1..4 problems per launch")
    f16 = problems[0].f16
    if any(pr.f16 != f16 for pr in problems):
        raise ValueError("conv_fused: all problems of a launch must use the same 16-bit operand type")
    arr = (ConvFParams * n)(*[pr.p for pr in problems])
    dev = problems[0].out.device
    key = (dev, torch.cuda.current_stream().cuda_stream)
    ws = _FUSED_WS.get(key)
    if ws is None:
        ws = _FUSED_WS[key] = torch.zeros(FUSED_WS_BYTES, device=dev, dtype=torch.uint8)
    if PROFILE_TAGS is not None:
        TAG[0] = "fused " + " + ".join(f"[{q.B}x{q.L}x{q.Cin}->{q.N} k{q.taps}{' up' + str(q.up_stride) if q.up_stride else ''}]" for q in (pr.p for pr in problems))
    _call("conv_tc", _lib.lib().b2a_conv1d_fused, 1, arr, n, 2 if TC_MODE[0] == "x2" else 1, int(f16), ws.data_ptr(), ws.numel(), _stream())
    return [pr.out for pr in problems]


def linear(x, cw: ConvW, *, planes=False, qkv_heads=0, qkv_scale=0.0, **kw):
    if planes or qkv_heads:
        if isinstance(x, torch.Tensor) and x.dim() != 3:
            raise ValueError("linear: planes= / qkv_heads= need a 3-D operand")
        B, L, _ = x.shape
        if not emit_tc_eligible(cw, L):
            raise ValueError("linear: planes= / qkv_heads= need a tensor-core layer (ops.emit_tc_eligible)")
        for k in ("out", "res"):
            t = kw.get(k)
            if t is not None and t.dim() == 2:
                kw[k] = t[None]
        out, pre, res = kw.pop("out", None), kw.pop("pre", None), kw.pop("res", None)
        post_act, post_p0, cscale, out_scale = kw.pop("post_act", 0), kw.pop("post_p0", 0.0), kw.pop("cscale", None), kw.pop("out_scale", 1.0)
        if kw:
            raise TypeError(f"linear: unsupported arguments with planes= / qkv_heads=: {sorted(kw)}")
        if isinstance(x, Planes) and (pre is not None or x.C != cw.cin or x.hi.shape[2] != cw.cin_pad or x.hi.dtype != torch.bfloat16):
            raise ValueError("linear: a Planes operand needs matching channels and dtype and takes no prologue")
        if out is None:
            out = torch.empty(B, L, cw.cout, device=cw.w.device, dtype=torch.float32)
        em = at = None
        if qkv_heads:
            if cw.cout != 3 * 64 * qkv_heads:
                raise ValueError(f"linear: qkv_heads={qkv_heads} needs Cout = {3 * 64 * qkv_heads}, got {cw.cout}")
            at = AttnPlanes(torch.empty(_lib.lib().b2a_attention_tc_ws_bytes(B, qkv_heads, L, L), device=out.device, dtype=torch.uint8),
                            B, L, qkv_heads)
        else:
            em = _new_planes(B, L, cw.cout, out.device)
        y = _conv1d_tc(x, cw, 1, 0, L, pre, post_act, post_p0, cscale, res, 1, out_scale, out, False, emit=em, attn=at, attn_scale=qkv_scale)
        return y, (at if qkv_heads else em)
    if isinstance(x, torch.Tensor) and x.dim() == 2:
        o = kw.get("out")
        if o is not None and o.dim() == 2:
            kw["out"] = o[None]
        r = kw.get("res")
        if r is not None and r.dim() == 2:
            kw["res"] = r[None]
        return conv1d(x[None], cw, **kw)[0]
    return conv1d(x, cw, **kw)


def copy2d(src: torch.Tensor, dst: torch.Tensor) -> None:
    rows, cols = src.shape
    assert dst.shape == src.shape and src.stride(1) == 1 and dst.stride(1) == 1
    _call("other", _lib.lib().b2a_copy2d, 1, src.data_ptr(), src.stride(0), dst.data_ptr(), dst.stride(0), rows, cols, _stream())


def stream_rows(entries) -> None:
    entries = [e for e in entries if e[0].numel()]
    if len(entries) > _lib.ROWOPS_MAX:
        raise ValueError(f"stream_rows: at most {_lib.ROWOPS_MAX} entries per launch, got {len(entries)}")
    if not entries:
        return
    arr = (_lib.RowOp * len(entries))()
    for i, (src, dst, add) in enumerate(entries):
        _chk3(src, "stream_rows src")
        _chk3(dst, "stream_rows dst")
        if src.shape != dst.shape:
            raise ValueError(f"stream_rows: source {tuple(src.shape)} and destination {tuple(dst.shape)} differ")
        B, rows, Cc = src.shape
        arr[i] = _lib.RowOp(src.data_ptr(), src.stride(0), src.stride(1), dst.data_ptr(), dst.stride(0), dst.stride(1), B, rows, Cc, int(bool(add)))
    _call("other", _lib.lib().b2a_stream_rows, 1, arr, len(entries), _stream())


def _stream_conv_params(x, cw: ConvW, B: int, L: int, lout: int, out, stride: int, dilation: int, pad_mode: int, pre: Optional[Pre],
                        post_act: int, res, res_div: int) -> Conv1dParams:
    p = Conv1dParams()
    if L:
        _chk3(x, "stream conv x")
        p.x, p.x_bs, p.x_ld = x.data_ptr(), x.stride(0), x.stride(1)
    p.B, p.L, p.Cin = B, L, cw.cin
    p.w, p.bias = cw.w.data_ptr(), _p(cw.bias)
    if lout:
        p.y, p.y_bs, p.y_ld = out.data_ptr(), out.stride(0), out.stride(1)
    p.Lout, p.Cout = lout, cw.cout
    p.K, p.stride, p.dilation, p.groups, p.pad_mode = cw.K, stride, dilation, cw.groups, pad_mode
    if pre is not None:
        if pre.scale is not None or pre.shift is not None or pre.a is not None or pre.b is not None:
            raise ValueError("stream conv: the prologue is an activation only")
        p.pre_act, p.pre_p0 = pre.act, pre.p0
    p.post_act = post_act
    if res is not None:
        _chk3(res, "stream conv res")
        p.res, p.res_bs, p.res_ld = res.data_ptr(), res.stride(0), res.stride(1)
    p.res_div, p.out_scale = res_div, 1.0
    return p


def conv1d_stream(x: Optional[torch.Tensor], cw: ConvW, hist: torch.Tensor, H: int, step: torch.Tensor, *, B=None, stride=1, dilation=1,
                  pad_mode=0, fresh=False, pre: Optional[Pre] = None, post_act=0, res=None, res_div=1, out=None) -> torch.Tensor:
    L = 0 if x is None else x.shape[1]
    B = x.shape[0] if x is not None else B
    keff = (cw.K - 1) * dilation + 1
    lout = (H + L - keff) // stride + 1 if H + L >= keff else 0
    if hist.dtype != torch.float32 or not hist.is_contiguous() or hist.shape != (2, B, max(keff - 1, 1), cw.cin):
        raise ValueError(f"conv1d_stream: history buffer must be float32 [2, {B}, {max(keff - 1, 1)}, {cw.cin}], got {tuple(hist.shape)}")
    if out is None:
        out = torch.empty(B, lout, cw.cout, device=hist.device, dtype=torch.float32)
    p = _stream_conv_params(x, cw, B, L, lout, out, stride, dilation, pad_mode, pre, post_act, res, res_div)
    _call("conv", _lib.lib().b2a_conv1d_stream, 1, C.byref(p), hist.data_ptr(), hist.stride(1), H, step.data_ptr(), int(fresh), _stream())
    return out


def convtr1d_stream(x: torch.Tensor, cw: ConvW, tail: torch.Tensor, *, stride: int, pre: Optional[Pre] = None, out=None) -> torch.Tensor:
    _chk3(x, "convtr1d_stream x")
    B, L, _ = x.shape
    if not tail.is_contiguous() or tail.shape != (B, cw.K - stride, cw.cout):
        raise ValueError(f"convtr1d_stream: tail must be contiguous [{B}, {cw.K - stride}, {cw.cout}], got {tuple(tail.shape)}")
    if out is None:
        out = torch.empty(B, L * stride, cw.cout, device=x.device, dtype=torch.float32)
    p = _stream_conv_params(x, cw, B, L, L * stride, out, stride, 1, 0, pre, 0, None, 1)
    _call("conv", _lib.lib().b2a_convtr1d_stream, 1, C.byref(p), tail.data_ptr(), tail.stride(0), _stream())
    return out


def ring_rope_kv(qkv: torch.Tensor, n_heads: int, k_ring: torch.Tensor, v_ring: torch.Tensor, pos: torch.Tensor, *, base: float) -> None:
    _chk3(qkv, "ring_rope_kv qkv")
    B, T, w = qkv.shape
    D = w // (3 * n_heads)
    _call("rope", _lib.lib().b2a_ring_rope_kv, 1, qkv.data_ptr(), qkv.stride(0), qkv.stride(1), B, T, n_heads, D, base, k_ring.data_ptr(),
          v_ring.data_ptr(), k_ring.stride(0), k_ring.shape[1], pos.data_ptr(), _stream())


def ring_attn(q: torch.Tensor, k_ring: torch.Tensor, v_ring: torch.Tensor, pos: torch.Tensor, *, n_heads: int, scale: float, window: int,
              out=None) -> torch.Tensor:
    _chk3(q, "ring_attn q")
    B, T, hd = q.shape
    if out is None:
        out = torch.empty(B, T, hd, device=q.device, dtype=torch.float32)
    _call("attention", _lib.lib().b2a_ring_attn, 1, q.data_ptr(), q.stride(0), q.stride(1), k_ring.data_ptr(), v_ring.data_ptr(), k_ring.stride(0),
          k_ring.shape[1], out.data_ptr(), out.stride(0), out.stride(1), B, T, n_heads, hd // n_heads, scale, window, pos.data_ptr(), _stream())
    return out


def stream_advance(ctr: torch.Tensor, dpos: int) -> None:
    assert ctr.dtype == torch.int32 and ctr.numel() >= 2
    _call("other", _lib.lib().b2a_stream_advance, 1, ctr.data_ptr(), dpos, _stream())


def gather_rows(src: torch.Tensor, idx: torch.Tensor, out: Optional[torch.Tensor] = None, add: Optional[torch.Tensor] = None) -> torch.Tensor:
    assert src.dim() == 2 and src.stride(1) == 1 and idx.dtype == torch.int64 and idx.is_contiguous()
    rows, cols = idx.shape[0], src.shape[1]
    if out is None:
        out = torch.empty(rows, cols, device=src.device, dtype=torch.float32)
    a, a_ld, a_per = (None, 0, 0) if add is None else (add.data_ptr(), add.stride(0), add.shape[0])
    _call("other", _lib.lib().b2a_gather_rows, 1, src.data_ptr(), src.stride(0), idx.data_ptr(), out.data_ptr(), out.stride(0),
          rows, cols, src.shape[0], a, a_ld, a_per, _stream())
    return out


def whisper_greedy_step(logits: torch.Tensor, tokens: torch.Tensor, cur_len: int, sample_begin: int, *, suppress_mask, blank_mask,
                        eot: int, no_timestamps: int, timestamp_begin: int, max_initial_ts: int, without_timestamps: bool,
                        sum_logprobs: torch.Tensor, not_done: torch.Tensor, temperature: float = 0.0, u: Optional[torch.Tensor] = None) -> torch.Tensor:
    B, V = logits.shape
    assert logits.stride(1) == 1 and tokens.dtype == torch.int64 and tokens.stride(1) == 1
    assert u is None or (u.dtype == torch.float32 and u.is_contiguous() and u.numel() == B)
    nxt = torch.empty(B, device=logits.device, dtype=torch.int64)
    _call("sampler", _lib.lib().b2a_whisper_greedy_step, 1, logits.data_ptr(), logits.stride(0), tokens.data_ptr(), tokens.stride(0), B, cur_len,
          sample_begin, V, _p(suppress_mask), _p(blank_mask), eot, no_timestamps, timestamp_begin, max_initial_ts, int(without_timestamps),
          nxt.data_ptr(), sum_logprobs.data_ptr(), not_done.data_ptr(), float(temperature), _p(u), _stream())
    return nxt


def durations_to_index(dur, max_frames: int, speed: float = 1.0):
    assert dur.is_contiguous() and dur.dtype in (torch.float32, torch.int64)
    T = dur.shape[0]
    pred = torch.empty(T, device=dur.device, dtype=torch.int64)
    idx = torch.zeros(max_frames, device=dur.device, dtype=torch.int64)
    total = torch.zeros(1, device=dur.device, dtype=torch.int64)
    f, i = (dur.data_ptr(), None) if dur.dtype == torch.float32 else (None, dur.data_ptr())
    _call("other", _lib.lib().b2a_durations_to_index, 1, f, i, T, speed, pred.data_ptr(), idx.data_ptr(), max_frames, total.data_ptr(), _stream())
    return pred, idx, total


_WS = {}


def _workspace(nbytes: int, device) -> torch.Tensor:
    key = (device, torch.cuda.current_stream().cuda_stream)
    ws = _WS.get(key)
    if ws is None or ws.numel() < nbytes:
        ws = torch.empty(max(nbytes, 1 << 20), device=device, dtype=torch.uint8)
        _WS[key] = ws
    return ws


def adain_coeffs(x: torch.Tensor, gb: Optional[torch.Tensor], eps=1e-5):
    _chk3(x, "adain_coeffs x")
    B, L, Cc = x.shape
    scale = torch.empty(B, Cc, device=x.device, dtype=torch.float32)
    shift = torch.empty(B, Cc, device=x.device, dtype=torch.float32)
    ws = _workspace(_lib.lib().b2a_adain_ws_bytes(B, L, Cc), x.device)
    _call("adain_stats", _lib.lib().b2a_adain_coeffs, 2, x.data_ptr(), x.stride(0), x.stride(1), B, L, Cc, _p(gb), eps,
                                           scale.data_ptr(), shift.data_ptr(), ws.data_ptr(), _stream())
    return scale, shift


def channel_stats(x: torch.Tensor, dsts) -> None:
    _chk3(x, "channel_stats x")
    B, L, Cc = x.shape
    if isinstance(dsts, torch.Tensor):
        dsts = [dsts]
    n = len(dsts)
    for d in dsts:
        assert d.dtype == torch.int64 and tuple(d.shape) == (B, Cc, 2, STAT_BINS) and d.stride(3) == 1 and d.stride(2) == STAT_BINS and d.stride(1) == 2 * STAT_BINS
    ptrs = (C.c_void_p * n)(*[d.data_ptr() for d in dsts])
    bss = (C.c_int64 * n)(*[d.stride(0) for d in dsts])
    _call("adain_stats", _lib.lib().b2a_channel_stats, 1, x.data_ptr(), x.stride(0), x.stride(1), B, L, Cc, ptrs, bss, n, _stream())


def coeffs_from_stats(stats: torch.Tensor, L: int, gb: Optional[torch.Tensor], eps=1e-5):
    B, Cc = stats.shape[:2]
    assert stats.dtype == torch.int64 and stats.is_contiguous() and tuple(stats.shape[2:]) == (2, STAT_BINS)
    scale = torch.empty(B, Cc, device=stats.device, dtype=torch.float32)
    shift = torch.empty(B, Cc, device=stats.device, dtype=torch.float32)
    _call("adain_stats", _lib.lib().b2a_coeffs_from_stats, 1, stats.data_ptr(), B, L, Cc, _p(gb), eps, scale.data_ptr(), shift.data_ptr(), _stream())
    return scale, shift


def layernorm(x: torch.Tensor, w=None, b=None, *, eps=1e-5, res=None, ada=None, rms=False, post_act=0, post_p0=0.0,
              out=None, planes=False):
    shp = x.shape
    x2 = x.reshape(-1, shp[-1]) if x.dim() != 2 else x
    assert x2.stride(1) == 1
    r2 = None
    if res is not None:
        r2 = res.reshape(-1, shp[-1]) if res.dim() != 2 else res
    if out is None:
        out = torch.empty(x2.shape, device=x.device, dtype=torch.float32)
    o2 = out.reshape(-1, shp[-1]) if out.dim() != 2 else out
    pl = None
    if planes:
        if shp[-1] % 64:
            raise ValueError(f"layernorm: planes=True needs C % 64 == 0, got {shp[-1]}")
        pl = _new_planes(1, x2.shape[0], shp[-1], x.device)
    _call("layernorm", _lib.lib().b2a_layernorm, 1, x2.data_ptr(), x2.stride(0), _p(r2), 0 if r2 is None else r2.stride(0), o2.data_ptr(),
                                        o2.stride(0), x2.shape[0], shp[-1], _p(w), _p(b), _p(ada), eps, int(rms), post_act,
                                        post_p0, None if pl is None else pl.hi.data_ptr(), None if pl is None else _p(pl.lo),
                                        shp[-1], _stream())
    y = out.reshape(shp) if out.dim() == 2 and len(shp) != 2 else out
    return (y, pl) if planes else y


def attention(q, k, v, *, n_heads, n_kv_heads=None, scale, causal=False, q_offset=0, window=0, k_len=None, out=None):
    for t, n in ((q, "q"), (k, "k"), (v, "v")):
        _chk3(t, "attention " + n)
    if window > 0 and not causal:
        raise ValueError(f"attention: a sliding window ({window}) needs causal=True")
    B, Tq, hd = q.shape
    H = n_heads
    Hkv = n_kv_heads or H
    D = hd // H
    if out is None:
        out = torch.empty(B, Tq, hd, device=q.device, dtype=torch.float32)
    p = AttnParams()
    p.q, p.k, p.v, p.o = q.data_ptr(), k.data_ptr(), v.data_ptr(), out.data_ptr()
    p.q_bs, p.q_ld, p.k_bs, p.k_ld = q.stride(0), q.stride(1), k.stride(0), k.stride(1)
    p.v_bs, p.v_ld, p.o_bs, p.o_ld = v.stride(0), v.stride(1), out.stride(0), out.stride(1)
    p.B, p.Tq, p.Tk, p.H, p.Hkv, p.D = B, Tq, k.shape[1], H, Hkv, D
    p.scale, p.causal, p.q_offset, p.window = scale, int(causal), q_offset, window
    p.k_len = _p(k_len)
    if ATTN_MODE[0] == "tc" and D == 64 and Hkv == H and k_len is None and k.shape[1] >= 64 and out.stride(1) % 4 == 0:
        ws = torch.empty(_lib.lib().b2a_attention_tc_ws_bytes(B, H, Tq, k.shape[1]), device=q.device, dtype=torch.uint8)
        _call("attention", _lib.lib().b2a_attention_tc, 4, C.byref(p), ws.data_ptr(), _stream())
        return out
    _call("attention", _lib.lib().b2a_attention, 1, C.byref(p), _stream())
    return out


_ALBERT_ERR = {}


def albert_error_word(device) -> torch.Tensor:
    device = torch.device(device)
    w = _ALBERT_ERR.get(device)
    if w is None:
        if torch.cuda.is_current_stream_capturing():
            raise RuntimeError("albert_encoder: run it once outside graph capture first (its error word is allocated then)")
        w = _ALBERT_ERR[device] = torch.zeros(1, device=device, dtype=torch.int32)
    return w


def albert_encoder(h: torch.Tensor, hp: Planes, layers: int, qkv: ConvW, attn_out: ConvW, ffn: ConvW, ffn_out: ConvW, ln_attn, ln_full,
                   *, heads: int, scale: float, eps: float, timeline: Optional[torch.Tensor] = None) -> None:
    if h.dtype != torch.float32 or not h.is_contiguous() or h.dim() != 3 or h.shape[0] != 1:
        raise ValueError(f"albert_encoder: h must be a contiguous float32 [1, T, hidden] tensor, got {tuple(h.shape)} {h.dtype}")
    T, hs = h.shape[1], h.shape[2]
    inter = ffn.cout
    for cw, (n, k) in ((qkv, (3 * hs, hs)), (attn_out, (hs, hs)), (ffn, (inter, hs)), (ffn_out, (hs, inter))):
        if cw.w_tc is None or cw.K != 1 or cw.f16 or cw.w_tc_lo is not None or (cw.cout, cw.cin_pad) != (n, k) or cw.bias is None:
            raise ValueError("albert_encoder: every projection needs bf16 tensor-core weights with a bias and matching shapes")
    two = TC_MODE[0] == "x2"
    if hp.hi.shape != (1, T, hs) or (hp.lo is not None) != two:
        raise ValueError("albert_encoder: hp must hold h's bf16 planes (hi, and lo in x2 mode)")
    a = _lib.AlbertParams()
    a.T, a.layers, a.heads, a.hidden, a.inter, a.planes = T, layers, heads, hs, inter, 2 if two else 1
    for i, cw in enumerate((qkv, attn_out, ffn, ffn_out)):
        a.w[i], a.bias[i] = cw.w_tc.data_ptr(), cw.bias.data_ptr()
    a.ln_w[0], a.ln_b[0] = ln_attn[0].data_ptr(), ln_attn[1].data_ptr()
    a.ln_w[1], a.ln_b[1] = ln_full[0].data_ptr(), ln_full[1].data_ptr()
    a.eps, a.scale = eps, scale
    a.h, a.h_hi, a.h_lo = h.data_ptr(), hp.hi.data_ptr(), _p(hp.lo)
    err = albert_error_word(h.device)
    ws = torch.empty(_lib.lib().b2a_albert_ws_bytes(T, heads, hs, inter), device=h.device, dtype=torch.uint8)
    _call("albert", _lib.lib().b2a_albert_encoder, 1, C.byref(a), ws.data_ptr(), err.data_ptr(), _p(timeline), _stream())


def attention_planes(ap: AttnPlanes, *, planes=False, out=None):
    B, T, H = ap.B, ap.T, ap.H
    if T < 64:
        raise ValueError("attention_planes: the tensor-core attention needs at least 64 keys")
    if out is None:
        out = torch.empty(B, T, H * 64, device=ap.ws.device, dtype=torch.float32)
    _chk3(out, "attention_planes out")
    pl = _new_planes(B, T, H * 64, out.device) if planes else None
    p = AttnParams()
    p.o, p.o_bs, p.o_ld = out.data_ptr(), out.stride(0), out.stride(1)
    p.B, p.Tq, p.Tk, p.H, p.Hkv, p.D = B, T, T, H, H, 64
    p.operands_ready = 1
    if pl is not None:
        p.emit_hi, p.emit_lo, p.emit_ld = pl.hi.data_ptr(), _p(pl.lo), H * 64
    _call("attention", _lib.lib().b2a_attention_tc, 1, C.byref(p), ap.ws.data_ptr(), _stream())
    return (out, pl) if planes else out


def rope_(x: torch.Tensor, n_heads: int, *, offset=0, base=10000.0, traditional=True) -> torch.Tensor:
    _chk3(x, "rope x")
    B, T, hd = x.shape
    _call("rope", _lib.lib().b2a_rope, 1, x.data_ptr(), x.stride(0), x.stride(1), B, T, n_heads, hd // n_heads, offset, base,
                                   int(traditional), _stream())
    return x


def lstm_bidir(xproj: torch.Tensor, wh: torch.Tensor, out: Optional[torch.Tensor] = None) -> torch.Tensor:
    B, T, g8 = xproj.shape
    H = g8 // 8
    assert xproj.is_contiguous() and wh.is_contiguous() and wh.shape == (2, 4 * H, H)
    if out is None:
        out = torch.empty(B, T, 2 * H, device=xproj.device, dtype=torch.float32)
    assert out.stride(2) == 1 and (B == 1 or out.stride(0) == T * out.stride(1))
    _call("lstm", _lib.lib().b2a_lstm_bidir, 1, xproj.data_ptr(), wh.data_ptr(), out.data_ptr(), out.stride(1), B, T, H, _stream())
    return out


def stft(x: torch.Tensor, window: torch.Tensor, n_fft: int, hop: int, pad_mode: int, frames: int):
    B, n = x.shape
    assert x.stride(1) == 1 and window.shape[0] == n_fft
    nf = n_fft // 2 + 1
    re = torch.empty(B, frames, nf, device=x.device, dtype=torch.float32)
    im = torch.empty(B, frames, nf, device=x.device, dtype=torch.float32)
    _call("other", _lib.lib().b2a_stft, 1, x.data_ptr(), x.stride(0), B, n, window.data_ptr(), n_fft, hop, pad_mode, frames,
                                   re.data_ptr(), im.data_ptr(), _stream())
    return re, im


def whisper_logmel(x: torch.Tensor, padding: int, window: torch.Tensor, filters: torch.Tensor, frames: int) -> torch.Tensor:
    B, n = x.shape
    assert x.stride(1) == 1 and filters.is_contiguous() and filters.shape[1] == 201
    out = torch.empty(B, frames, filters.shape[0], device=x.device, dtype=torch.float32)
    gmax = torch.empty(B, device=x.device, dtype=torch.float32)
    _call("logmel", _lib.lib().b2a_whisper_logmel, 2, x.data_ptr(), x.stride(0), B, n, padding, window.data_ptr(), filters.data_ptr(),
                                             filters.shape[0], frames, out.data_ptr(), gmax.data_ptr(), _stream())
    return out


def istft(re: torch.Tensor, im: torch.Tensor, n_fft: int, hop: int, window: torch.Tensor, *, norm_sq: bool, clamp_mode: int,
          trim: int, out_len: int) -> torch.Tensor:
    B, nf, T = re.shape
    assert re.is_contiguous() and im.is_contiguous() and nf == n_fft // 2 + 1
    out = torch.empty(B, out_len, device=re.device, dtype=torch.float32)
    ws = torch.empty(B, T, n_fft, device=re.device, dtype=torch.float32)
    _call("other", _lib.lib().b2a_istft, 2, re.data_ptr(), im.data_ptr(), B, n_fft, T, hop, window.data_ptr(), int(norm_sq), clamp_mode,
                                    trim, out_len, out.data_ptr(), ws.data_ptr(), _stream())
    return out


def resample_poly(x: torch.Tensor, h: torch.Tensor, up: int, down: int, n_pre_pad: int, n_pre_remove: int, n_out: int) -> torch.Tensor:
    assert x.dim() == 2 and x.stride(1) == 1 and h.dtype == torch.float64 and h.is_contiguous()
    out = torch.empty(x.shape[0], n_out, device=x.device, dtype=torch.float32)
    _call("resample", _lib.lib().b2a_resample_poly, 1, x.data_ptr(), x.stride(0), x.shape[0], x.shape[1], h.data_ptr(), h.shape[0], up, down,
          n_pre_pad, n_pre_remove, out.data_ptr(), n_out, _stream())
    return out


def kokoro_source(f0: torch.Tensor, noise: Optional[torch.Tensor], lin_w: torch.Tensor, lin_b: torch.Tensor) -> torch.Tensor:
    B, nF = f0.shape
    assert f0.is_contiguous()
    har = torch.empty(B, nF * 60 + 1, 22, device=f0.device, dtype=torch.float32)
    src = torch.empty(B, nF * 300, device=f0.device, dtype=torch.float32)
    n_down = max(1, int(math.ceil(float(nF * 300) * float(1 / 300))))
    ph = torch.empty(B, n_down, 9, device=f0.device, dtype=torch.float64)
    if noise is not None:
        assert noise.is_contiguous() and noise.shape == (B, nF * 300, 9)
    _call("source", _lib.lib().b2a_kokoro_source, 3, f0.data_ptr(), B, nF, n_down, _p(noise), lin_w.data_ptr(), lin_b.data_ptr(), har.data_ptr(),
                                            src.data_ptr(), ph.data_ptr(), _stream())
    return har


def kokoro_source_conv(har: torch.Tensor, cw: ConvW, *, stride: int = 1, pad_left: int = 0) -> torch.Tensor:
    _chk3(har, "kokoro_source_conv har")
    B, L, cin = har.shape
    if cin != 22 or cw.cin != 22 or cw.groups != 1 or not har.is_contiguous():
        raise ValueError("kokoro_source_conv: expected a contiguous [B, L, 22] source and a dense 22-channel layer")
    lout = (L + 2 * pad_left - cw.K) // stride + 1
    out = torch.empty(B, lout, cw.cout, device=har.device, dtype=torch.float32)
    if PROFILE_TAGS is not None:
        TAG[0] = f"source conv [{B}x{L}x{cin}->{cw.cout} k{cw.K} s{stride}]"
    _call("conv" if cin * cw.K >= 64 else "other", _lib.lib().b2a_kokoro_source_conv, 1, har.data_ptr(), B, L, cw.w.data_ptr(), _p(cw.bias),
          out.data_ptr(), lout, cw.cout, cw.K, stride, pad_left, _stream())
    return out


def kokoro_istft_head(x: torch.Tensor) -> torch.Tensor:
    _chk3(x, "kokoro_istft_head x")
    B, T, _ = x.shape
    audio = torch.empty(B, (T - 1) * 5, device=x.device, dtype=torch.float32)
    _call("istft_head", _lib.lib().b2a_kokoro_istft_head, 1, x.data_ptr(), x.stride(0), x.stride(1), B, T, audio.data_ptr(), _stream())
    return audio


def randn_(out: torch.Tensor, seed: int, offset: int = 0) -> torch.Tensor:
    assert out.is_contiguous() and out.dtype == torch.float32
    _call("other", _lib.lib().b2a_randn, 1, out.data_ptr(), out.numel(), seed, offset, _stream())
    return out


def randn_dev_(out: torch.Tensor, state: torch.Tensor) -> torch.Tensor:
    assert out.is_contiguous() and out.dtype == torch.float32 and state.dtype == torch.int64 and state.numel() == 2 and state.is_contiguous()
    _call("other", _lib.lib().b2a_randn_dev, 2, out.data_ptr(), out.numel(), state.data_ptr(), _stream())
    return out


def sample_token(logits: torch.Tensor, *, temperature: float, top_k: int = 0, top_p: float = 1.0, min_p: float = 0.0, u=None,
                 suppress_mask=None, seen=None, repetition_penalty: float = 1.0, return_filtered: bool = False, mark_seen: bool = False,
                 out: Optional[torch.Tensor] = None, finished=None, eos: int = -1):
    B, V = logits.shape
    assert logits.stride(1) == 1 and (seen is None or (seen.dtype == torch.uint8 and seen.stride(1) == 1))
    if out is None:
        out = torch.empty(B, device=logits.device, dtype=torch.int64)
    assert out.dtype == torch.int64 and out.dim() == 1 and out.shape[0] == B
    filt = torch.empty(B, V, device=logits.device, dtype=torch.float32) if return_filtered else None
    _call("sampler", _lib.lib().b2a_sample_token, 1, logits.data_ptr(), logits.stride(0), B, V, _p(suppress_mask), _p(seen),
          0 if seen is None else seen.stride(0), int(mark_seen), repetition_penalty, temperature, top_k, top_p, min_p, _p(u),
          out.data_ptr(), out.stride(0) if B > 1 else 1, _p(filt), _p(finished), eos, _stream())
    return (out, filt) if return_filtered else out


def gemv_eligible(cw: "ConvW") -> bool:
    return cw.K == 1 and cw.w_tc is not None and not cw.f16 and cw.w_tc_lo is None and cw.cin % 8 == 0


def gemv(x: torch.Tensor, cw: "ConvW", *, norm_w=None, norm_eps: float = 1e-6, swiglu: bool = False, res=None, out=None,
         prefetch: Optional["ConvW"] = None) -> torch.Tensor:
    if not (x.dim() == 2 and x.stride(1) == 1 and gemv_eligible(cw)):
        raise NotImplementedError("gemv needs a bf16-exact K=1 weight with Cout % 32 == 0 and Cin % 8 == 0 (see ops.gemv_eligible); "
                                  "use ops.linear")
    M, K = x.shape
    N = cw.cout
    n_out = N // 2 if swiglu else N
    if out is None:
        out = torch.empty(M, n_out, device=x.device, dtype=torch.float32)
    assert K == cw.cin and out.shape == (M, n_out) and out.stride(1) == 1
    pf, pf_bytes = (None, 0) if prefetch is None or prefetch.w_tc is None else (prefetch.w_tc.data_ptr(), prefetch.w_tc.numel() * 2)
    for m0 in range(0, M, 8):
        m = min(8, M - m0)
        r = None if res is None else res[m0:m0 + m]
        _call("gemv", _lib.lib().b2a_gemv_bf16, 1, x[m0:m0 + m].data_ptr(), x.stride(0), m, K, cw.w_tc.data_ptr(), cw.cin_pad, N,
              _p(cw.bias), _p(norm_w), norm_eps, int(swiglu), _p(r), 0 if r is None else r.stride(0), out[m0:m0 + m].data_ptr(),
              out.stride(0), pf if m0 == 0 else None, pf_bytes, _stream())
    return out


def qknorm_rope_cache(qkv: torch.Tensor, n_heads: int, n_kv: int, head_dim: int, k_cache: torch.Tensor, v_cache: torch.Tensor, *,
                      q_norm=None, k_norm=None, eps: float = 1e-6, pos3=None, base_dev=None, base: int = 0, mrope=(0, 0),
                      theta: float = 10000.0, q_out=None, pos_shift=None, base_rows=None, slot=None) -> torch.Tensor:
    _chk3(qkv, "qkv")
    B, S, _ = qkv.shape
    if q_out is None:
        q_out = torch.empty(B, S, n_heads * head_dim, device=qkv.device, dtype=torch.float32)
    assert k_cache.shape == v_cache.shape and k_cache.stride() == v_cache.stride() and k_cache.stride(2) == 1
    assert pos3 is None or (pos3.dtype == torch.int32 and pos3.is_contiguous() and pos3.shape == (3, B, S))
    _call("rope", _lib.lib().b2a_qknorm_rope_cache, 1, qkv.data_ptr(), qkv.stride(0), qkv.stride(1), B, S, n_heads, n_kv, head_dim,
          _p(q_norm), _p(k_norm), eps, _p(pos3), _p(base_dev), base, mrope[0], mrope[1], theta, q_out.data_ptr(), q_out.stride(0),
          q_out.stride(1), k_cache.data_ptr(), v_cache.data_ptr(), k_cache.stride(0), k_cache.stride(1), k_cache.shape[1], _p(pos_shift),
          _p(_rows_i32(base_rows, B)), _p(_rows_i32(slot, B)), _stream())
    return q_out


def attn_decode(q: torch.Tensor, k_cache: torch.Tensor, v_cache: torch.Tensor, n_heads: int, n_kv: int, head_dim: int, *, scale: float,
                base_dev=None, base: int = 0, kv_start=None, max_k: Optional[int] = None, out=None, base_rows=None, slot=None) -> torch.Tensor:
    _chk3(q, "q")
    B, S, _ = q.shape
    if out is None:
        out = torch.empty(B, S, n_heads * head_dim, device=q.device, dtype=torch.float32)
    if max_k is None:
        max_k = k_cache.shape[1] if base_dev is not None or base_rows is not None else base + S
    _call("attention", _lib.lib().b2a_attn_decode, 1, q.data_ptr(), q.stride(0), q.stride(1), k_cache.data_ptr(), v_cache.data_ptr(),
          k_cache.stride(0), k_cache.stride(1), out.data_ptr(), out.stride(0), out.stride(1), B, S, n_heads, n_kv, head_dim, scale,
          _p(base_dev), base, _p(kv_start), max_k, _p(_rows_i32(base_rows, B)), _p(_rows_i32(slot, B)), _stream())
    return out


def attn_prefill(q: torch.Tensor, k_cache: torch.Tensor, v_cache: torch.Tensor, n_heads: int, n_kv: int, head_dim: int, *, scale: float,
                 base_dev=None, base: int = 0, kv_start=None, max_k: Optional[int] = None, out=None, base_rows=None, slot=None) -> torch.Tensor:
    _chk3(q, "q")
    B, S, _ = q.shape
    if out is None:
        out = torch.empty(B, S, n_heads * head_dim, device=q.device, dtype=torch.float32)
    if max_k is None:
        max_k = k_cache.shape[1] if base_dev is not None or base_rows is not None else base + S
    _call("attention", _lib.lib().b2a_attn_prefill, 1, q.data_ptr(), q.stride(0), q.stride(1), k_cache.data_ptr(), v_cache.data_ptr(),
          k_cache.stride(0), k_cache.stride(1), out.data_ptr(), out.stride(0), out.stride(1), B, S, n_heads, n_kv, head_dim, scale,
          _p(base_dev), base, _p(kv_start), max_k, _p(_rows_i32(base_rows, B)), _p(_rows_i32(slot, B)), _stream())
    return out


def swiglu(x: torch.Tensor, out=None, interleaved: bool = False) -> torch.Tensor:
    shp = x.shape
    I = shp[-1] // 2
    x2 = x.reshape(-1, shp[-1])
    assert x2.stride(1) == 1
    if out is None:
        out = torch.empty(*shp[:-1], I, device=x.device, dtype=torch.float32)
    o2 = out.reshape(-1, I)
    _call("other", _lib.lib().b2a_swiglu, 1, x2.data_ptr(), x2.stride(0), x2.shape[0], I, int(interleaved), o2.data_ptr(), o2.stride(0), _stream())
    return out


class EmbedTables:

    def __init__(self, tables):
        self.tables = [t for t in tables]
        for t in self.tables:
            assert t.dim() == 2 and t.is_contiguous() and t.dtype == torch.float32 and t.shape[1] == self.tables[0].shape[1]
        dev = self.tables[0].device
        self.ptrs = torch.tensor([t.data_ptr() for t in self.tables], dtype=torch.int64, device=dev)
        self.bins = torch.tensor([t.shape[0] for t in self.tables], dtype=torch.int32, device=dev)
        self.dim = self.tables[0].shape[1]


def embed_sum(codes: torch.Tensor, tabs: EmbedTables, *, text=None, pad=None, step_dev=None, step_sub: int = 0, out=None, err=None,
              tidx=None, finished=None) -> torch.Tensor:
    assert codes.dtype == torch.int64 and codes.dim() == 2 and codes.stride(1) == 1
    B, G = codes.shape
    assert G <= len(tabs.tables)
    if out is None:
        out = torch.empty(B, tabs.dim, device=codes.device, dtype=torch.float32)
    tb, ts, nt = (0, 0, 0) if text is None else (text.stride(0), text.stride(1), text.shape[1])
    _call("other", _lib.lib().b2a_embed_sum, 1, codes.data_ptr(), codes.stride(0), B, G, tabs.dim, tabs.ptrs.data_ptr(), tabs.bins.data_ptr(),
          _p(text), tb, ts, nt, _p(pad), _p(step_dev), step_sub, out.data_ptr(), out.stride(0), _p(err), _p(tidx), _p(finished), _stream())
    return out


def _rows_i32(t: Optional[torch.Tensor], B: int) -> Optional[torch.Tensor]:
    assert t is None or (t.dtype == torch.int32 and t.is_cuda and t.is_contiguous() and t.numel() == B), "per-row arrays are int32 [B] on the device"
    return t


def slot_advance(lengths: torch.Tensor, frames: torch.Tensor, finished: torch.Tensor, cap: torch.Tensor, codes: torch.Tensor,
                 out: torch.Tensor, u_tab: torch.Tensor, u: torch.Tensor) -> None:
    B, G = codes.shape
    assert codes.dtype == torch.int64 and codes.is_contiguous() and out.dtype == torch.int64 and out.is_contiguous() and out.shape[0] == B
    assert finished.dtype == torch.uint8 and all(t.dtype == torch.int32 and t.numel() == B for t in (lengths, frames, cap))
    assert u_tab.is_contiguous() and u_tab.shape[0] == B and u.is_contiguous() and u.shape == (G, B)
    _call("other", _lib.lib().b2a_slot_advance, 1, lengths.data_ptr(), frames.data_ptr(), finished.data_ptr(), cap.data_ptr(), codes.data_ptr(),
          G, out.data_ptr(), out.stride(0), u_tab.data_ptr(), u_tab.stride(0), u.data_ptr(), B, _stream())


def incr_(p: torch.Tensor, v: int = 1) -> None:
    assert p.dtype == torch.int32
    _call("other", _lib.lib().b2a_incr_i32, 1, p.data_ptr(), v, _stream())


def rvq_decode(codes: torch.Tensor, codebooks: torch.Tensor, out: Optional[torch.Tensor] = None, check=True,
               err: Optional[torch.Tensor] = None) -> torch.Tensor:
    assert codes.dtype == torch.int64 and (codes.stride(2) == 1 or codes.shape[2] == 1) and codebooks.is_contiguous()
    B, nq, T = codes.shape
    _, bins, dim = codebooks.shape
    if out is None:
        out = torch.empty(B, T, dim, device=codes.device, dtype=torch.float32)
    if err is None:
        err = torch.zeros(1, device=codes.device, dtype=torch.int32)
    _call("rvq", _lib.lib().b2a_rvq_decode, 1, codes.data_ptr(), codes.stride(0), codes.stride(1), B, nq, T, codebooks.data_ptr(), bins,
                                         dim, out.data_ptr(), out.stride(1), err.data_ptr(), _stream())
    if check and int(err.item()) != 0:
        raise ValueError(f"rvq_decode: code index out of range [0, {bins})")
    return out


def rvq_encode(x: torch.Tensor, codebooks: torch.Tensor, c2: torch.Tensor, *, mode: int = 0, out: Optional[torch.Tensor] = None) -> torch.Tensor:
    assert x.dim() == 2 and x.stride(1) == 1 and x.dtype == torch.float32 and codebooks.is_contiguous() and c2.dtype == torch.float64 and c2.is_contiguous()
    R, D = x.shape
    nq, bins, _ = codebooks.shape
    if out is None:
        out = torch.empty(R, nq, device=x.device, dtype=torch.int64)
    assert out.shape == (R, nq) and out.dtype == torch.int64
    _call("rvq", _lib.lib().b2a_rvq_encode, 1, x.data_ptr(), x.stride(0), R, D, codebooks.data_ptr(), c2.data_ptr(), bins, nq, mode, out.data_ptr(),
          out.stride(0), out.stride(1), _stream())
    return out


def snac_from_codes(codes, strides, embs, ws, biases, dim: int, check=True) -> torch.Tensor:
    n = len(codes)
    B = codes[0].shape[0]
    T = codes[-1].shape[1] * strides[-1]
    bins, cd = embs[0].shape
    out = torch.empty(B, T, dim, device=codes[0].device, dtype=torch.float32)
    err = torch.zeros(1, device=out.device, dtype=torch.int32)
    arr = lambda ts: (C.c_void_p * n)(*[None if t is None else t.data_ptr() for t in ts])
    for c in codes:
        assert c.dtype == torch.int64 and c.is_contiguous()
    _call("rvq", _lib.lib().b2a_snac_from_codes, 1, arr(codes), (C.c_int32 * n)(*strides), n, arr(embs), arr(ws), arr(biases), B, T, bins,
                                              cd, dim, out.data_ptr(), err.data_ptr(), _stream())
    if check and int(err.item()) != 0:
        raise ValueError(f"snac_from_codes: code index out of range [0, {bins})")
    return out


def dac_levels(levels, device) -> torch.Tensor:
    arr = (_lib.DacLevel * len(levels))()
    off = 0
    for a, lv in zip(arr, levels):
        for k in ("w_in", "b_in", "cbn", "c2", "cb", "w_out", "b_out"):
            t = lv.get(k)
            assert t is None or (t.is_cuda and t.is_contiguous() and t.dtype == (torch.float64 if k == "c2" else torch.float32))
            setattr(a, k, _p(t))
        a.cd, a.lat_off = lv["cb"].shape[1], off
        off += a.cd
    return torch.frombuffer(bytearray(bytes(arr)), dtype=torch.uint8).to(device)


def dac_rvq_encode(z: Optional[torch.Tensor], table: torch.Tensor, n_levels: int, bins: int, lat_ch: int, dim: int, *,
                   latents: Optional[torch.Tensor] = None):
    if z is not None:
        _chk3(z, "dac_rvq_encode z")
        assert z.is_contiguous() and z.shape[2] == dim
        B, T, _ = z.shape
        latents = torch.empty(B, lat_ch, T, device=z.device, dtype=torch.float32)
    else:
        assert latents.dtype == torch.float32 and latents.is_cuda and latents.is_contiguous() and latents.shape[1] == lat_ch
        B, _, T = latents.shape
    dev = latents.device
    codes = torch.empty(B, n_levels, T, device=dev, dtype=torch.int64)
    zq = torch.empty(B, T, dim, device=dev, dtype=torch.float32)
    loss = torch.empty(-(-B * T // 8), device=dev, dtype=torch.float64)
    _call("rvq", _lib.lib().b2a_dac_rvq_encode, 1, _p(z), dim, B, T, dim, table.data_ptr(), n_levels, bins, lat_ch, codes.data_ptr(),
          latents.data_ptr(), zq.data_ptr(), loss.data_ptr(), _stream())
    return codes, latents, zq, loss


def dac_from_codes(codes: torch.Tensor, table: torch.Tensor, bins: int, lat_ch: int, dim: int, *, want_zp=False, check=True):
    assert codes.dtype == torch.int64 and codes.is_cuda and codes.dim() == 3 and (codes.stride(2) == 1 or codes.shape[2] == 1)
    B, nq, T = codes.shape
    out = torch.empty(B, T, dim, device=codes.device, dtype=torch.float32)
    zp = torch.empty(B, lat_ch, T, device=codes.device, dtype=torch.float32) if want_zp else None
    err = torch.zeros(1, device=codes.device, dtype=torch.int32)
    _call("rvq", _lib.lib().b2a_dac_from_codes, 1, codes.data_ptr(), codes.stride(0), codes.stride(1), B, nq, T, table.data_ptr(), bins, lat_ch,
          dim, out.data_ptr(), _p(zp), err.data_ptr(), _stream())
    if check and int(err.item()) != 0:
        raise ValueError(f"dac_from_codes: code index out of range [0, {bins})")
    return out, zp


def aa_snakebeta(x: torch.Tensor, a: torch.Tensor, inv_b: torch.Tensor, f_up: torch.Tensor, f_down: torch.Tensor, *,
                 planes_for: Optional[ConvW] = None):
    _chk3(x, "aa_snakebeta x")
    B, L, Cc = x.shape
    for name, t, n in (("a", a, Cc), ("inv_b", inv_b, Cc), ("f_up", f_up, f_up.numel()), ("f_down", f_down, f_down.numel())):
        if t.dtype != torch.float32 or not t.is_cuda or not t.is_contiguous() or t.numel() != n:
            raise ValueError(f"aa_snakebeta: {name} must be a contiguous CUDA float32 tensor of {n} values")
    if f_up.numel() != f_down.numel():
        raise ValueError("aa_snakebeta: the up- and down-sampling filters must have the same number of taps")
    if planes_for is not None:
        if planes_for.cin != Cc or planes_for.w_tc is None or planes_for.f16:
            raise ValueError("aa_snakebeta: planes_for must be a bf16 tensor-core conv taking the activation's channels")
        out = _new_planes(B, L, planes_for.cin_pad, x.device)
        out.C = Cc
        _call("aa_act", _lib.lib().b2a_aa_snakebeta, 1, x.data_ptr(), x.stride(0), x.stride(1), B, L, Cc, a.data_ptr(), inv_b.data_ptr(),
              f_up.data_ptr(), f_down.data_ptr(), 2, f_up.numel(), None, 0, 0, out.hi.data_ptr(), _p(out.lo), planes_for.cin_pad, _stream())
        return out
    out = torch.empty(B, L, Cc, device=x.device, dtype=torch.float32)
    _call("aa_act", _lib.lib().b2a_aa_snakebeta, 1, x.data_ptr(), x.stride(0), x.stride(1), B, L, Cc, a.data_ptr(), inv_b.data_ptr(),
          f_up.data_ptr(), f_down.data_ptr(), 2, f_up.numel(), out.data_ptr(), out.stride(0), out.stride(1), None, None, 0, _stream())
    return out


def spk_logmel(x: torch.Tensor, window: torch.Tensor, filters: torch.Tensor) -> torch.Tensor:
    B, n = x.shape
    assert x.dtype == torch.float32 and x.stride(1) == 1 and window.numel() == 1024 and filters.is_contiguous() and filters.shape[1] == 513
    if n <= 384:
        raise ValueError(f"speaker log-mel: the reflect padding of 384 samples needs more than 384 samples, got {n}")
    frames = 1 + (n + 768 - 1024) // 256
    out = torch.empty(B, frames, filters.shape[0], device=x.device, dtype=torch.float32)
    _call("logmel", _lib.lib().b2a_spk_logmel, 1, x.data_ptr(), x.stride(0), B, n, window.data_ptr(), filters.data_ptr(), filters.shape[0],
          frames, out.data_ptr(), _stream())
    return out


def spk_reflect_pad(x: torch.Tensor, pad: int, cpad: int = 0, planes: int = 2):
    _chk3(x, "spk_reflect_pad x")
    B, T, Cc = x.shape
    if pad >= T:
        raise ValueError(f"reflect padding of {pad} rows needs more than {pad} frames, got {T}")
    if cpad:
        pl = Planes(torch.empty(B, T + 2 * pad, cpad, device=x.device, dtype=torch.bfloat16),
                    torch.empty(B, T + 2 * pad, cpad, device=x.device, dtype=torch.bfloat16) if planes == 2 else None, Cc)
        _call("prep", _lib.lib().b2a_spk_reflect_pad, 1, x.data_ptr(), x.stride(0), x.stride(1), B, T, Cc, pad, None, pl.hi.data_ptr(),
              _p(pl.lo), cpad, _stream())
        return pl
    out = torch.empty(B, T + 2 * pad, Cc, device=x.device, dtype=torch.float32)
    _call("prep", _lib.lib().b2a_spk_reflect_pad, 1, x.data_ptr(), x.stride(0), x.stride(1), B, T, Cc, pad, out.data_ptr(), None, None, 0,
          _stream())
    return out


SPK_RES2NET_TILE = 32


def spk_res2net(y: torch.Tensor, w: torch.Tensor, bias: torch.Tensor, scale: int, dilation: int, out=None, tile: int = 0) -> torch.Tensor:
    _chk3(y, "spk_res2net y")
    B, T, CC = y.shape
    S1, K, Cc, _ = w.shape
    assert S1 == scale - 1 and CC == scale * Cc and w.is_contiguous() and bias.is_contiguous() and w.dtype == torch.float32
    pad = (K - 1) * dilation // 2
    if pad >= T:
        raise ValueError(f"Res2Net: reflect padding of {pad} rows needs more than {pad} frames, got {T}")
    if out is None:
        out = torch.empty(B, T, CC, device=y.device, dtype=torch.float32)
    _chk3(out, "spk_res2net out")
    _call("other", _lib.lib().b2a_spk_res2net, 1, y.data_ptr(), y.stride(0), y.stride(1), out.data_ptr(), out.stride(0), out.stride(1),
          w.data_ptr(), bias.data_ptr(), B, T, Cc, scale, K, dilation, tile or SPK_RES2NET_TILE, _stream())
    return out


def spk_channel_stats(x: torch.Tensor, with_std: bool, eps: float = 1e-12, out=None) -> torch.Tensor:
    _chk3(x, "spk_channel_stats x")
    B, T, Cc = x.shape
    if out is None:
        out = torch.empty(B, (2 if with_std else 1) * Cc, device=x.device, dtype=torch.float32)
    _call("other", _lib.lib().b2a_spk_channel_stats, 1, x.data_ptr(), x.stride(0), x.stride(1), B, T, Cc, int(with_std), eps,
          out.data_ptr(), out.stride(0), _stream())
    return out


def spk_se_gate(mean: torch.Tensor, w1, b1, w2, b2) -> torch.Tensor:
    B, Cc = mean.shape
    S = w1.shape[0]
    assert mean.stride(1) == 1 and w1.is_contiguous() and w2.is_contiguous() and tuple(w2.shape) == (Cc, S)
    gate = torch.empty(B, Cc, device=mean.device, dtype=torch.float32)
    _call("other", _lib.lib().b2a_spk_se_gate, 1, mean.data_ptr(), mean.stride(0), B, Cc, S, w1.data_ptr(), b1.data_ptr(), w2.data_ptr(),
          b2.data_ptr(), gate.data_ptr(), _stream())
    return gate


def spk_se_apply(y: torch.Tensor, gate: torch.Tensor, res: torch.Tensor, out: torch.Tensor) -> torch.Tensor:
    for t, n in ((y, "y"), (res, "res"), (out, "out")):
        _chk3(t, "spk_se_apply " + n)
    B, T, Cc = y.shape
    assert res.shape == y.shape and out.shape == y.shape and gate.is_contiguous() and tuple(gate.shape) == (B, Cc)
    _call("other", _lib.lib().b2a_spk_se_apply, 1, y.data_ptr(), y.stride(0), y.stride(1), gate.data_ptr(), res.data_ptr(), res.stride(0),
          res.stride(1), out.data_ptr(), out.stride(0), out.stride(1), B, T, Cc, _stream())
    return out


def spk_gemv(x: torch.Tensor, w: torch.Tensor, bias: Optional[torch.Tensor] = None, act: int = 0) -> torch.Tensor:
    B, K = x.shape
    N = w.shape[0]
    assert x.stride(1) == 1 and w.stride(1) == 1 and w.shape[1] == K and x.dtype == w.dtype == torch.float32
    y = torch.empty(B, N, device=x.device, dtype=torch.float32)
    _call("gemv", _lib.lib().b2a_spk_gemv, 1, x.data_ptr(), x.stride(0), B, K, w.data_ptr(), w.stride(0), N, _p(bias), act, y.data_ptr(),
          y.stride(0), _stream())
    return y


def spk_asp_act(h: torch.Tensor, cb: torch.Tensor) -> torch.Tensor:
    _chk3(h, "spk_asp_act h")
    B, T, A = h.shape
    assert cb.is_contiguous() and tuple(cb.shape) == (B, A)
    _call("other", _lib.lib().b2a_spk_asp_act, 1, h.data_ptr(), h.stride(0), h.stride(1), cb.data_ptr(), B, T, A, _stream())
    return h


def spk_asp_pool(logits: torch.Tensor, x: torch.Tensor, eps: float = 1e-12) -> torch.Tensor:
    _chk3(logits, "spk_asp_pool logits")
    _chk3(x, "spk_asp_pool x")
    B, T, Cc = x.shape
    assert logits.shape == x.shape
    out = torch.empty(B, 2 * Cc, device=x.device, dtype=torch.float32)
    _call("other", _lib.lib().b2a_spk_asp_pool, 1, logits.data_ptr(), logits.stride(0), logits.stride(1), x.data_ptr(), x.stride(0),
          x.stride(1), B, T, Cc, eps, out.data_ptr(), out.stride(0), _stream())
    return out


def vocos_dwnorm(x: torch.Tensor, dw: Optional[ConvW], w: Optional[torch.Tensor], b: Optional[torch.Tensor], *, ada: Optional[torch.Tensor] = None,
                 eps: float = 1e-6, fp32: bool = True, planes: bool = False):
    _chk3(x, "vocos_dwnorm x")
    B, L, Cc = x.shape
    if not (fp32 or planes):
        raise ValueError("vocos_dwnorm: ask for fp32 rows, planes or both")
    if dw is not None and (dw.groups != Cc or dw.cin != Cc or dw.K % 2 == 0 or dw.K > 15):
        raise ValueError("vocos_dwnorm: dw must be a depthwise conv over x's channels with an odd number of taps <= 15")
    if ada is not None and (ada.dim() != 2 or ada.shape[0] != B or ada.shape[1] != 2 * Cc or ada.stride(1) != 1 or ada.dtype != torch.float32):
        raise ValueError(f"vocos_dwnorm: ada must be float32 [B, 2C] = {(B, 2 * Cc)} rows with unit column stride")
    y = torch.empty(B, L, Cc, device=x.device, dtype=torch.float32) if fp32 else None
    pl = _new_planes(B, L, Cc, x.device) if planes else None
    _call("vocos_norm", _lib.lib().b2a_vocos_dwnorm, 1, x.data_ptr(), x.stride(0), x.stride(1), B, L, Cc,
          None if dw is None else dw.w.data_ptr(), None if dw is None else _p(dw.bias), 0 if dw is None else dw.K, _p(w), _p(b), _p(ada),
          0 if ada is None else ada.stride(0), float(eps), _p(y), 0 if y is None else y.stride(0), 0 if y is None else y.stride(1),
          None if pl is None else pl.hi.data_ptr(), None if pl is None else _p(pl.lo), _stream())
    if fp32 and planes:
        return y, pl
    return y if fp32 else pl


def vocos_istft_head(h: torch.Tensor, n_fft: int, hop: int, window: torch.Tensor) -> torch.Tensor:
    _chk3(h, "vocos_istft_head h")
    B, T, ld = h.shape
    if ld < n_fft + 2 or window.numel() != n_fft or window.dtype != torch.float32 or not window.is_contiguous():
        raise ValueError(f"vocos_istft_head: needs h rows of >= {n_fft + 2} columns and a contiguous float32 window of {n_fft}")
    out = torch.empty(B, (T - 1) * hop, device=h.device, dtype=torch.float32)
    if T > 1:
        _call("vocos_head", _lib.lib().b2a_vocos_istft_head, 1, h.data_ptr(), h.stride(0), h.stride(1), B, T, n_fft, hop, window.data_ptr(),
              out.data_ptr(), out.stride(0), _stream())
    return out


def vocos_logmel(x: torch.Tensor, window: torch.Tensor, filters: torch.Tensor) -> torch.Tensor:
    B, n = x.shape
    if x.dtype != torch.float32 or x.stride(1) != 1 or window.numel() != 1024 or not filters.is_contiguous() or filters.shape[1] != 513:
        raise ValueError("vocos_logmel: x [B, n] float32 with unit stride, a 1024-sample window and [n_mels, 513] filters")
    if n <= 512:
        raise ValueError(f"vocos log-mel: the reflect padding of 512 samples needs more than 512 samples, got {n}")
    frames = n // 256
    out = torch.empty(B, frames, filters.shape[0], device=x.device, dtype=torch.float32)
    _call("logmel", _lib.lib().b2a_vocos_logmel, 1, x.data_ptr(), x.stride(0), B, n, window.data_ptr(), filters.data_ptr(), filters.shape[0],
          frames, out.data_ptr(), _stream())
    return out


def encodec_lstm(xproj: torch.Tensor, wh: torch.Tensor, err: torch.Tensor, skip: Optional[torch.Tensor] = None) -> torch.Tensor:
    R, T, g4 = xproj.shape
    H = g4 // 4
    for name, t in (("xproj", xproj), ("wh", wh)) + ((("skip", skip),) if skip is not None else ()):
        if t.dtype != torch.float32 or not t.is_cuda or not t.is_contiguous():
            raise ValueError(f"encodec_lstm: {name} must be a contiguous CUDA float32 tensor")
    if tuple(wh.shape) != (4 * H, H) or (skip is not None and tuple(skip.shape) != (R, T, H)):
        raise ValueError(f"encodec_lstm: wh must be [{4 * H}, {H}] and skip [{R}, {T}, {H}]")
    out = torch.empty(R, T, H, device=xproj.device, dtype=torch.float32)
    _call("lstm", _lib.lib().b2a_encodec_lstm, 1, xproj.data_ptr(), wh.data_ptr(), _p(skip), out.data_ptr(), R, T, H, err.data_ptr(), _stream())
    return out


def encodec_pad(x: torch.Tensor, pad_left: int, pad_right: int, *, reflect: bool = True, coeffs=None, elu: bool = False,
                res: Optional[torch.Tensor] = None) -> torch.Tensor:
    _chk3(x, "encodec_pad x")
    B, T, Cc = x.shape
    if reflect and max(pad_left, pad_right) >= T:
        raise ValueError(f"EnCodec reflect padding ({pad_left}, {pad_right}) needs more than {max(pad_left, pad_right)} frames, got {T}")
    out = torch.empty(B, pad_left + T + pad_right, Cc, device=x.device, dtype=torch.float32)
    sc, sh = coeffs if coeffs is not None else (None, None)
    if res is not None:
        _chk3(res, "encodec_pad res")
    _call("prep", _lib.lib().b2a_encodec_pad, 1, x.data_ptr(), x.stride(0), x.stride(1), B, T, Cc, pad_left, pad_right, int(reflect), _p(sc),
          _p(sh), int(elu), _p(res), 0 if res is None else res.stride(0), 0 if res is None else res.stride(1), out.data_ptr(), out.stride(0),
          out.stride(1), _stream())
    return out


def encodec_gn_coeffs(x: torch.Tensor, gamma: Optional[torch.Tensor], beta: Optional[torch.Tensor], eps: float = 1e-5):
    _chk3(x, "encodec_gn_coeffs x")
    B, T, Cc = x.shape
    scale = torch.empty(B, Cc, device=x.device, dtype=torch.float32)
    shift = torch.empty(B, Cc, device=x.device, dtype=torch.float32)
    ws = _workspace(_lib.lib().b2a_encodec_gn_ws_bytes(B), x.device)
    _call("norm", _lib.lib().b2a_encodec_gn_coeffs, 2, x.data_ptr(), x.stride(0), x.stride(1), B, T, Cc, _p(gamma), _p(beta), eps,
          scale.data_ptr(), shift.data_ptr(), ws.data_ptr(), _stream())
    return scale, shift


def encodec_normalize(x: torch.Tensor, mask: Optional[torch.Tensor]):
    _chk3(x, "encodec_normalize x")
    R, L, Cc = x.shape
    if mask is not None:
        assert mask.dtype in (torch.bool, torch.uint8) and tuple(mask.shape) == (R, L) and mask.stride(1) == 1
    y = torch.empty(R, L, Cc, device=x.device, dtype=torch.float32)
    scale = torch.empty(R, device=x.device, dtype=torch.float32)
    _call("other", _lib.lib().b2a_encodec_normalize, 1, x.data_ptr(), x.stride(0), x.stride(1), R, L, Cc, _p(mask),
          0 if mask is None else mask.stride(0), y.data_ptr(), scale.data_ptr(), _stream())
    return y, scale


def encodec_ola(frames: torch.Tensor, B: int, scale: Optional[torch.Tensor], stride: int, t_out: int) -> torch.Tensor:
    NB, L, Cc = frames.shape
    assert frames.dtype == torch.float32 and frames.is_contiguous() and NB % B == 0
    assert scale is None or (scale.dtype == torch.float32 and scale.is_contiguous() and scale.numel() == NB)
    out = torch.empty(B, t_out, Cc, device=frames.device, dtype=torch.float32)
    _call("other", _lib.lib().b2a_encodec_ola, 1, frames.data_ptr(), NB // B, B, L, Cc, _p(scale), stride, t_out, out.data_ptr(), _stream())
    return out


def lm_sample_mlx(logits: torch.Tensor, *, temperature: float, top_p: float, u: Optional[torch.Tensor] = None,
                  step_dev: Optional[torch.Tensor] = None, out: Optional[torch.Tensor] = None, hist: Optional[torch.Tensor] = None,
                  finished: Optional[torch.Tensor] = None, stop_ids=()) -> torch.Tensor:
    B, V = logits.shape
    if logits.dtype != torch.float32 or not logits.is_cuda or logits.stride(1) != 1:
        raise ValueError("lm_sample_mlx: logits must be a CUDA float32 [B, V] tensor with unit column stride")
    if temperature > 0 and (u is None or u.dtype != torch.float32 or u.dim() != 2 or u.shape[0] != B or u.stride(1) != 1):
        raise ValueError("lm_sample_mlx: temperature > 0 needs float32 uniforms u [B, steps]")
    stops = [int(s) for s in stop_ids if s is not None]
    if len(stops) > 2:
        raise ValueError("lm_sample_mlx: at most two stop ids")
    stops += [-1] * (2 - len(stops))
    if out is None:
        out = torch.empty(B, device=logits.device, dtype=torch.int64)
    assert out.dtype == torch.int64 and out.is_contiguous() and out.numel() == B
    assert step_dev is None or (step_dev.dtype == torch.int32 and step_dev.is_cuda)
    assert hist is None or (hist.dtype == torch.int64 and hist.dim() == 2 and hist.stride(1) == 1 and hist.shape[0] == B)
    assert finished is None or (finished.dtype == torch.uint8 and finished.is_contiguous() and finished.numel() == B)
    _call("sampler", _lib.lib().b2a_lm_sample_mlx, 1, logits.data_ptr(), logits.stride(0), B, V, float(temperature), float(top_p), _p(u),
          0 if u is None else u.stride(0), _p(step_dev), out.data_ptr(), _p(hist), 0 if hist is None else hist.stride(0), _p(finished),
          stops[0], stops[1], _stream())
    return out


def soprano_upsample(x: torch.Tensor, up: int, *, planes_for: Optional[ConvW] = None):
    _chk3(x, "soprano_upsample x")
    B, L, H = x.shape
    Lo = up * (L - 1) + 1
    if planes_for is not None:
        if planes_for.cin != H or planes_for.w_tc is None or planes_for.f16:
            raise ValueError("soprano_upsample: planes_for must be a bf16 tensor-core conv taking the hidden width")
        out = _new_planes(B, Lo, planes_for.cin_pad, x.device)
        out.C = H
        _call("other", _lib.lib().b2a_soprano_upsample, 1, x.data_ptr(), x.stride(0), x.stride(1), B, L, H, up, None, 0, 0,
              out.hi.data_ptr(), _p(out.lo), planes_for.cin_pad, _stream())
        return out
    out = torch.empty(B, Lo, H, device=x.device, dtype=torch.float32)
    _call("other", _lib.lib().b2a_soprano_upsample, 1, x.data_ptr(), x.stride(0), x.stride(1), B, L, H, up, out.data_ptr(), out.stride(0),
          out.stride(1), None, None, 0, _stream())
    return out


def store_rows_at(src: torch.Tensor, dst: torch.Tensor, idx_dev: torch.Tensor, add: int = 0) -> None:
    B, H = src.shape
    assert src.dtype == dst.dtype == torch.float32 and src.stride(1) == 1 and dst.stride(2) == 1 and dst.shape[0] == B and dst.shape[2] == H
    assert idx_dev.dtype == torch.int32 and idx_dev.is_cuda
    _call("other", _lib.lib().b2a_soprano_store_rows, 1, src.data_ptr(), src.stride(0), B, H, dst.data_ptr(), dst.stride(0), dst.stride(1),
          idx_dev.data_ptr(), int(add), dst.shape[1], _stream())
```

Measured before the change: 1837.

## Replace grid-wide barriers in ALBERT megakernel with per-row-block dataflow counters

The persistent ALBERT encoder kernel used to wait on a grid-wide barrier between every stage. It now splits the CTAs into groups that each own interleaved 64-row blocks and orders each unit's work by per-stage, per-row-block arrival counters, so a row block moves to its next stage once its own inputs are ready. Attention operands are double-buffered by layer parity so the next layer's QKV can overlap the current layer's attention, and the grid size becomes configurable. This removes global synchronisation stalls and load imbalance, at the cost of more complex indexing, a larger workspace, and possible deadlock or ordering bugs.

New measurement: 1851, median of 6. About the same (+0.7%).

```diff
diff --git a/include/b200audio.h b/include/b200audio.h
--- a/include/b200audio.h
+++ b/include/b200audio.h
@@ -83,8 +83,10 @@
   const float* ln_b[2];
   float eps, scale;
   float* h; void* h_hi; void* h_lo;
+  int32_t grid;
 } b2a_albert_t;
 int64_t b2a_albert_ws_bytes(int32_t T, int32_t heads, int32_t hidden, int32_t inter);
+int32_t b2a_albert_ws_regions(int32_t T, int32_t heads, int32_t hidden, int32_t inter, int64_t* out);
 int32_t b2a_albert_encoder(const b2a_albert_t* a, void* ws, uint32_t* err, int64_t* timeline, void* stream);
 
 int32_t b2a_conv1d_tc_debug(void* dbg8);
diff --git a/mlx_audio_b200/_lib.py b/mlx_audio_b200/_lib.py
--- a/mlx_audio_b200/_lib.py
+++ b/mlx_audio_b200/_lib.py
@@ -59,7 +59,7 @@
 class AlbertParams(C.Structure):
     _fields_ = [("T", i32), ("layers", i32), ("heads", i32), ("hidden", i32), ("inter", i32), ("planes", i32),
                 ("w", C.c_void_p * 4), ("bias", C.c_void_p * 4), ("ln_w", C.c_void_p * 2), ("ln_b", C.c_void_p * 2),
-                ("eps", f32), ("scale", f32), ("h", C.c_void_p), ("h_hi", C.c_void_p), ("h_lo", C.c_void_p)]
+                ("eps", f32), ("scale", f32), ("h", C.c_void_p), ("h_hi", C.c_void_p), ("h_lo", C.c_void_p), ("grid", i32)]
 
 
 class RowOp(C.Structure):
@@ -104,6 +104,7 @@
     "b2a_attention_tc_ws_bytes": (i64, [i32, i32, i32, i32]),
     "b2a_attention_tc": (i32, [C.POINTER(AttnParams), C.c_void_p, C.c_void_p]),
     "b2a_albert_ws_bytes": (i64, [i32, i32, i32, i32]),
+    "b2a_albert_ws_regions": (i32, [i32, i32, i32, i32, C.c_void_p]),
     "b2a_albert_encoder": (i32, [C.POINTER(AlbertParams), C.c_void_p, C.c_void_p, C.c_void_p, C.c_void_p]),
     "b2a_rope": (i32, [c_f, i64, i64, i32, i32, i32, i32, i32, f32, i32, C.c_void_p]),
     "b2a_lstm_bidir": (i32, [c_f, c_f, c_f, i64, i32, i32, i32, C.c_void_p]),
diff --git a/mlx_audio_b200/csrc/albert.cu b/mlx_audio_b200/csrc/albert.cu
--- a/mlx_audio_b200/csrc/albert.cu
+++ b/mlx_audio_b200/csrc/albert.cu
@@ -16,6 +16,11 @@
 constexpr int OFF_BAR = OFF_Q + 2 * PLANE;
 constexpr int SMEM_BYTES = OFF_BAR + (2 * SLOTS + 2) * 8 + 16 + 1024;
 constexpr int STAGES = 7;
+constexpr int LN_ROWS = 8;
+constexpr int MAX_MB = 8;
+enum { C_ATT, C_AO, C_LN1, C_FFN, C_FO, C_LN2, C_N };
+constexpr int CNT_BYTES = 256;
+static_assert((MAX_MB + C_N * MAX_MB) * 4 <= CNT_BYTES, "counters outside the memset");
 constexpr long long TIMEOUT_NS = 10000000000LL;
 
 struct AlbertMaps {
@@ -33,11 +38,61 @@
   __nv_bfloat16 *hp_hi, *hp_lo, *ap_hi, *ap_lo, *fp_hi, *fp_lo;
   __nv_bfloat16 *cp_hi, *cp_lo;
   AttnOperands attn;
-  unsigned* bar; unsigned* err;
+  int ng;
+  int ulayer, ustart[STAGES + 1], ncol[STAGES];
+  unsigned* cnt; unsigned* err;
   long long* tl;
 };
 
 __device__ __forceinline__ int gemm_of_stage(int s) { return s == 0 ? 0 : s == 2 ? 1 : s == 4 ? 2 : s == 5 ? 3 : -1; }
+__device__ __forceinline__ unsigned* counter(const AlbertParams& p, int c, int m) { return p.cnt + MAX_MB + c * MAX_MB + m; }
+
+struct Group { int g, nb, rank, size; };
+__device__ __forceinline__ Group group_of(const AlbertParams& p) {
+  Group gr;
+  const int c = blockIdx.x, grid = gridDim.x;
+  gr.g = ((c + 1) * p.ng - 1) / grid;
+  const int start = gr.g * grid / p.ng;
+  gr.nb = (p.mb - gr.g + p.ng - 1) / p.ng;
+  gr.rank = c - start;
+  gr.size = (gr.g + 1) * grid / p.ng - start;
+  return gr;
+}
+
+struct Unit { int l, s, m, col; };
+__device__ __forceinline__ Unit unit_of(const AlbertParams& p, int q) {
+  const Group gr = group_of(p);
+  Unit u;
+  const int per_layer = gr.nb * p.ulayer;
+  u.l = q / per_layer;
+  int r = q - u.l * per_layer;
+  u.s = 0;
+#pragma unroll
+  for (int s = 1; s < STAGES; s++) u.s += r >= gr.nb * p.ustart[s];
+  r -= gr.nb * p.ustart[u.s];
+  const int b = r / p.ncol[u.s];
+  u.col = r - b * p.ncol[u.s];
+  u.m = gr.g + b * p.ng;
+  return u;
+}
+
+__device__ __forceinline__ int opaque(int v) { asm volatile("mov.b32 %0, %0;" : "+r"(v)); return v; }
+
+struct Dep { const unsigned* c; unsigned target; };
+__device__ __forceinline__ Dep dep_of(const AlbertParams& p, int l, int s, int m) {
+  switch (s) {
+    case 0: return {l ? counter(p, C_LN2, m) : nullptr, (unsigned)l * (64 / LN_ROWS)};
+    case 1: return {p.cnt, (unsigned)(l + 1) * p.mb * (p.N[0] / 64)};
+    case 2: return {counter(p, C_ATT, m), (unsigned)(l + 1) * p.H};
+    case 3: return {counter(p, C_AO, m), (unsigned)(l + 1) * (p.hs / 64)};
+    case 4: return {counter(p, C_LN1, m), (unsigned)(l + 1) * (64 / LN_ROWS)};
+    case 5: return {counter(p, C_FFN, m), (unsigned)(l + 1) * (p.inter / 64)};
+    default: return {counter(p, C_FO, m), (unsigned)(l + 1) * (p.hs / 64)};
+  }
+}
+__device__ __forceinline__ unsigned* arrival_of(const AlbertParams& p, int s, int m) {
+  return s == 0 ? p.cnt : counter(p, s - 1, m);
+}
 
 __device__ __forceinline__ long long globaltimer() {
   long long t;
@@ -45,11 +100,11 @@
   return t;
 }
 
-__device__ bool grid_wait(const AlbertParams& p, unsigned target) {
+__device__ bool dep_wait(const AlbertParams& p, const unsigned* c, unsigned target) {
   long long t0 = 0;
   for (int it = 0;; it++) {
     unsigned v;
-    asm volatile("ld.acquire.gpu.global.u32 %0, [%1];" : "=r"(v) : "l"(p.bar) : "memory");
+    asm volatile("ld.acquire.gpu.global.u32 %0, [%1];" : "=r"(v) : "l"(c) : "memory");
     if ((int)(v - target) >= 0) return true;
     if ((it & 63) == 63) {
       if (*(volatile unsigned*)p.err) return false;
@@ -61,8 +116,8 @@
   }
 }
 
-__device__ __forceinline__ void grid_arrive(unsigned* bar) {
-  asm volatile("red.release.gpu.global.add.u32 [%0], 1;" ::"l"(bar) : "memory");
+__device__ __forceinline__ void arrive(unsigned* c) {
+  asm volatile("red.release.gpu.global.add.u32 [%0], 1;" ::"l"(c) : "memory");
 }
 
 __device__ __forceinline__ void fence_proxy_async_global() { asm volatile("fence.proxy.async.global;" ::: "memory"); }
@@ -76,8 +131,8 @@
   uint64_t* q_full = empty + SLOTS;
   uint64_t* q_empty = q_full + 1;
   const int warp = threadIdx.x >> 5, lane = threadIdx.x & 31;
-  const int bid = blockIdx.x, grid = gridDim.x;
-  const int total = p.layers * STAGES;
+  const Group grp = group_of(p);
+  const int total = p.layers * grp.nb * p.ulayer;
 
   if (warp == 8 && lane == 0) {
     for (int g = 0; g < 4; g++) {
@@ -94,71 +149,69 @@
   if (warp == 8) {
     if (lane != 0) return;
     uint32_t g = 0, qn = 0;
-    for (int k = 0; k < total; k++) {
-      const int stage = k % STAGES, gi = gemm_of_stage(stage);
-      if (stage == 1) {
-        const int units = p.H * p.mb;
-        if (bid >= units) continue;
-        grid_wait(p, (unsigned)k * grid);
-        fence_proxy_async_global();
-        for (int u = bid; u < units; u += grid) {
-          const int head = u / p.mb, q0 = (u % p.mb) * 64;
-          mbar_wait(q_empty, (qn & 1) ^ 1);
-          mbar_expect_tx(q_full, 2 * PLANE);
-          tma_load_3d(smem + OFF_Q, &maps.qh, q_full, 0, q0, head);
-          tma_load_3d(smem + OFF_Q + PLANE, &maps.ql, q_full, 0, q0, head);
-          qn++;
-          for (int t = 0; t < p.nkt; t++, g++) {
-            const int s = g % SLOTS;
-            uint8_t* st = smem + (size_t)s * SLOT_BYTES;
-            mbar_wait(empty + s, ((g / SLOTS) & 1) ^ 1);
-            mbar_expect_tx(full + s, 4 * PLANE);
-            tma_load_3d(st, &maps.kh, full + s, 0, t * 64, head);
-            tma_load_3d(st + PLANE, &maps.kl, full + s, 0, t * 64, head);
-            tma_load_3d(st + 2 * PLANE, &maps.vh, full + s, t * 64, 0, head);
-            tma_load_3d(st + 3 * PLANE, &maps.vl, full + s, t * 64, 0, head);
-          }
+    int att_layer = -1;
+    for (int G = grp.rank; G < total; G += grp.size) {
+      const Unit un = unit_of(p, G);
+      const int gi = gemm_of_stage(un.s), m0 = un.m * 64;
+      if (un.s == 3 || un.s == 6) continue;
+      if (gi < 0) {
+        if (att_layer != un.l) {
+          const Dep d = dep_of(p, un.l, 1, 0);
+          dep_wait(p, d.c, d.target);
+          fence_proxy_async_global();
+          att_layer = un.l;
+        }
+        const int head = (un.l & 1) * p.H + un.col;
+        mbar_wait(q_empty, (qn & 1) ^ 1);
+        mbar_expect_tx(q_full, 2 * PLANE);
+        tma_load_3d(smem + OFF_Q, &maps.qh, q_full, 0, m0, head);
+        tma_load_3d(smem + OFF_Q + PLANE, &maps.ql, q_full, 0, m0, head);
+        qn++;
+        for (int t = 0; t < p.nkt; t++, g++) {
+          const int s = g % SLOTS;
+          uint8_t* st = smem + (size_t)s * SLOT_BYTES;
+          mbar_wait(empty + s, ((g / SLOTS) & 1) ^ 1);
+          mbar_expect_tx(full + s, 4 * PLANE);
+          tma_load_3d(st, &maps.kh, full + s, 0, t * 64, head);
+          tma_load_3d(st + PLANE, &maps.kl, full + s, 0, t * 64, head);
+          tma_load_3d(st + 2 * PLANE, &maps.vh, full + s, t * 64, 0, head);
+          tma_load_3d(st + 3 * PLANE, &maps.vl, full + s, t * 64, 0, head);
         }
         continue;
       }
-      if (gi < 0) continue;
-      const int units = p.mb * (p.N[gi] / 64), kc = p.K[gi] / 64;
+      const int kc = p.K[gi] / 64, n0 = un.col * 64;
       const uint32_t bytes = (uint32_t)(PLANE * p.planes + PLANE);
-      bool waited = k == 0;
-      for (int u = bid; u < units; u += grid) {
-        const int m0 = (u % p.mb) * 64, n0 = (u / p.mb) * 64;
-        int pre = 0;
-        if (!waited) {
-          pre = kc < SLOTS ? kc : SLOTS;
-          for (int c = 0; c < pre; c++) {
-            const uint32_t gc = g + c;
-            const int s = gc % SLOTS;
-            mbar_wait(empty + s, ((gc / SLOTS) & 1) ^ 1);
-            mbar_expect_tx(full + s, bytes);
-            tma_load_2d(smem + (size_t)s * SLOT_BYTES + 2 * PLANE, &maps.w[gi], full + s, c * 64, n0);
-          }
-          grid_wait(p, (unsigned)k * grid);
-          fence_proxy_async_global();
-          waited = true;
-          for (int c = 0; c < pre; c++) {
-            const int s = (g + c) % SLOTS;
-            uint8_t* st = smem + (size_t)s * SLOT_BYTES;
-            tma_load_2d(st, &maps.a_hi[gi], full + s, c * 64, m0);
-            if (p.planes == 2) tma_load_2d(st + PLANE, &maps.a_lo[gi], full + s, c * 64, m0);
-          }
-        }
-        for (int c = pre; c < kc; c++) {
+      const Dep d = dep_of(p, un.l, un.s, un.m);
+      int pre = 0;
+      if (d.c) {
+        pre = kc < SLOTS ? kc : SLOTS;
+        for (int c = 0; c < pre; c++) {
           const uint32_t gc = g + c;
           const int s = gc % SLOTS;
-          uint8_t* st = smem + (size_t)s * SLOT_BYTES;
           mbar_wait(empty + s, ((gc / SLOTS) & 1) ^ 1);
           mbar_expect_tx(full + s, bytes);
-          tma_load_2d(st + 2 * PLANE, &maps.w[gi], full + s, c * 64, n0);
+          tma_load_2d(smem + (size_t)s * SLOT_BYTES + 2 * PLANE, &maps.w[gi], full + s, c * 64, n0);
+        }
+        dep_wait(p, d.c, d.target);
+        fence_proxy_async_global();
+        for (int c = 0; c < pre; c++) {
+          const int s = (g + c) % SLOTS;
+          uint8_t* st = smem + (size_t)s * SLOT_BYTES;
           tma_load_2d(st, &maps.a_hi[gi], full + s, c * 64, m0);
           if (p.planes == 2) tma_load_2d(st + PLANE, &maps.a_lo[gi], full + s, c * 64, m0);
         }
-        g += kc;
-      }
+      }
+      for (int c = pre; c < kc; c++) {
+        const uint32_t gc = g + c;
+        const int s = gc % SLOTS;
+        uint8_t* st = smem + (size_t)s * SLOT_BYTES;
+        mbar_wait(empty + s, ((gc / SLOTS) & 1) ^ 1);
+        mbar_expect_tx(full + s, bytes);
+        tma_load_2d(st + 2 * PLANE, &maps.w[gi], full + s, c * 64, n0);
+        tma_load_2d(st, &maps.a_hi[gi], full + s, c * 64, m0);
+        if (p.planes == 2) tma_load_2d(st + PLANE, &maps.a_lo[gi], full + s, c * 64, m0);
+      }
+      g += kc;
     }
     return;
   }
@@ -166,128 +219,145 @@
   const int ct = threadIdx.x, wg = warp >> 2, w4 = warp & 3;
   const uint32_t sb = smem_u32(smem);
   uint32_t g = 0, qn = 0;
-  for (int k = 0; k < total; k++) {
-    const int stage = k % STAGES, gi = gemm_of_stage(stage);
-    if (k > 0) {
-      if (ct == 0) grid_wait(p, (unsigned)k * grid);
+  for (int G = grp.rank; G < total; G += grp.size) {
+    const Unit un = unit_of(p, G);
+    const int gi = gemm_of_stage(un.s), m0 = un.m * 64;
+    long long t0 = 0;
+    if constexpr (TL) { if (ct == 0) t0 = globaltimer(); }
+    {
+      const Dep d = dep_of(p, un.l, un.s, un.m);
+      if (ct == 0 && d.c) dep_wait(p, d.c, d.target);
       bar_sync(1, 256);
     }
-    if constexpr (TL) { if (ct == 0) p.tl[((int64_t)k * grid + bid) * 2] = globaltimer(); }
+    if constexpr (TL) {
+      if (ct == 0) {
+        long long* r = p.tl + ((int64_t)(un.l * STAGES + un.s) * gridDim.x + blockIdx.x) * 3;
+        if (r[0] == 0) r[0] = t0;
+        r[2] += globaltimer() - t0;
+      }
+    }
     if (gi >= 0) {
-      const int units = p.mb * (p.N[gi] / 64), kc = p.K[gi] / 64, N = p.N[gi];
+      const int kc = p.K[gi] / 64, N = p.N[gi], n0 = un.col * 64;
       const float* bias = p.bias[gi];
-      for (int u = bid; u < units; u += grid) {
-        const int m0 = (u % p.mb) * 64, n0 = (u / p.mb) * 64;
-        float acc[16];
-        int prev = -1;
-        for (int c = 0; c < kc; c++, g++) {
-          const int s = g % SLOTS;
-          mbar_wait(full + s, (g / SLOTS) & 1);
-          const uint32_t st = sb + s * SLOT_BYTES;
-          const uint64_t ad = gmma_desc_sw128(st), wd = gmma_desc_sw128(st + 2 * PLANE + wg * 32 * 128);
-          wgmma_fence();
-          wgmma_chunk<1, false>(acc, ad, wd, c != 0);
-          if (p.planes == 2) wgmma_chunk<1, false>(acc, gmma_desc_sw128(st + PLANE), wd, 1u);
-          wgmma_commit();
-          wgmma_wait<1>();
-          wgmma_fence_regs<16>(acc);
-          if (prev >= 0 && (ct & 127) == 0) mbar_arrive(empty + prev);
-          prev = s;
-        }
-        wgmma_wait<0>();
+      float acc[16];
+      int prev = -1;
+      for (int c = 0; c < kc; c++, g++) {
+        const int s = g % SLOTS;
+        mbar_wait(full + s, (g / SLOTS) & 1);
+        const uint32_t st = sb + s * SLOT_BYTES;
+        const uint64_t ad = gmma_desc_sw128(st), wd = gmma_desc_sw128(st + 2 * PLANE + wg * 32 * 128);
+        wgmma_fence();
+        wgmma_chunk<1, false>(acc, ad, wd, c != 0);
+        if (p.planes == 2) wgmma_chunk<1, false>(acc, gmma_desc_sw128(st + PLANE), wd, 1u);
+        wgmma_commit();
+        wgmma_wait<1>();
         wgmma_fence_regs<16>(acc);
-        if ((ct & 127) == 0) mbar_arrive(empty + prev);
+        if (prev >= 0 && (ct & 127) == 0) mbar_arrive(empty + prev);
+        prev = s;
+      }
+      wgmma_wait<0>();
+      wgmma_fence_regs<16>(acc);
+      if ((ct & 127) == 0) mbar_arrive(empty + prev);
 #pragma unroll
-        for (int j = 0; j < 4; j++) {
-          const int n = n0 + wg * 32 + 8 * j + 2 * (lane & 3);
-          const float b0 = __ldg(bias + n), b1 = __ldg(bias + n + 1);
-          EmitCol e0{}, e1{};
-          if (gi == 0) { e0 = emit_col_attn(p.attn, 0, p.T, p.hs, p.qmul, n); e1 = emit_col_attn(p.attn, 0, p.T, p.hs, p.qmul, n + 1); }
+      for (int j = 0; j < 4; j++) {
+        const int n = n0 + wg * 32 + 8 * j + 2 * (lane & 3);
+        const float b0 = __ldg(bias + n), b1 = __ldg(bias + n + 1);
+        EmitCol e0{}, e1{};
+        if (gi == 0) {
+          const int64_t hb = (un.l & 1) * p.H;
+          e0 = emit_col_attn(p.attn, hb, p.T, p.hs, p.qmul, n);
+          e1 = emit_col_attn(p.attn, hb, p.T, p.hs, p.qmul, n + 1);
+        }
 #pragma unroll
-          for (int hh = 0; hh < 2; hh++) {
-            const int row = m0 + 16 * w4 + (lane >> 2) + 8 * hh;
-            const float a0 = acc[4 * j + 2 * hh], a1 = acc[4 * j + 2 * hh + 1];
-            if (row >= p.T) {
-              if (gi == 0 && e0.step == 1 && row < p.attn.tkp) { e0.hi[row] = 0; e0.lo[row] = 0; e1.hi[row] = 0; e1.lo[row] = 0; }
-              continue;
-            }
-            const int64_t o = (int64_t)row * N + n;
-            if (gi == 0) {
-              emit_store(e0, row, epilogue_value(a0, b0, 0, 0.f, 1.f, 0.f));
-              emit_store(e1, row, epilogue_value(a1, b1, 0, 0.f, 1.f, 0.f));
-            } else if (gi == 2) {
-              const float y0 = epilogue_value(a0, b0, B2A_ACT_GELU, 0.f, 1.f, 0.f), y1 = epilogue_value(a1, b1, B2A_ACT_GELU, 0.f, 1.f, 0.f);
-              __nv_bfloat162 h2, l2;
-              split16(y0, h2.x, l2.x);
-              split16(y1, h2.y, l2.y);
-              *reinterpret_cast<__nv_bfloat162*>(p.fp_hi + o) = h2;
-              if (p.planes == 2) *reinterpret_cast<__nv_bfloat162*>(p.fp_lo + o) = l2;
-            } else {
-              const float* res = gi == 1 ? p.h : p.t;
-              float* out = gi == 1 ? p.t : p.u;
-              const float2 r = *reinterpret_cast<const float2*>(res + o);
-              *reinterpret_cast<float2*>(out + o) = make_float2(epilogue_value(a0, b0, 0, 0.f, 1.f, r.x), epilogue_value(a1, b1, 0, 0.f, 1.f, r.y));
-            }
+        for (int hh = 0; hh < 2; hh++) {
+          const int row = m0 + 16 * w4 + (lane >> 2) + 8 * hh;
+          const float a0 = acc[4 * j + 2 * hh], a1 = acc[4 * j + 2 * hh + 1];
+          if (row >= p.T) {
+            if (gi == 0 && e0.step == 1 && row < p.attn.tkp) { e0.hi[row] = 0; e0.lo[row] = 0; e1.hi[row] = 0; e1.lo[row] = 0; }
+            continue;
           }
-        }
-      }
-    } else if (stage == 1) {
-      const int units = p.H * p.mb;
-      for (int u = bid; u < units; u += grid, qn++) {
-        const int head = u / p.mb, q0 = (u % p.mb) * 64;
-        float o[32], m[2] = {-INFINITY, -INFINITY}, l[2] = {0.f, 0.f};
-#pragma unroll
-        for (int j = 0; j < 32; j++) o[j] = 0.f;
-        const int kmax[2] = {p.T - 1, p.T - 1}, kmin[2] = {0, 0};
-        const uint64_t dqh = gmma_desc_sw128(sb + OFF_Q), dql = gmma_desc_sw128(sb + OFF_Q + PLANE);
-        mbar_wait(q_full, qn & 1);
-        for (int t = 0; t < p.nkt; t++, g++) {
-          const int s = g % SLOTS;
-          const uint32_t st = sb + s * SLOT_BYTES;
-          mbar_wait(full + s, (g / SLOTS) & 1);
-          if (wg == 0)
-            attn_tc_tile(o, m, l, dqh, dql, gmma_desc_sw128(st), gmma_desc_sw128(st + PLANE), gmma_desc_sw128(st + 2 * PLANE),
-                         gmma_desc_sw128(st + 3 * PLANE), t * 64, kmax, kmin, lane);
-          if ((ct & 127) == 0) mbar_arrive(empty + s);
-        }
-        if ((ct & 127) == 0) mbar_arrive(q_empty);
-        if (wg == 0) {
-          float inv[2];
-          attn_tc_row_inv(l, inv);
-#pragma unroll
-          for (int hh = 0; hh < 2; hh++) {
-            const int q = q0 + w4 * 16 + (lane >> 2) + 8 * hh;
-            if (q < p.T) {
-              const int64_t e = (int64_t)q * p.hs + head * 64 + 2 * (lane & 3);
-#pragma unroll
-              for (int j = 0; j < 8; j++) {
-                __nv_bfloat162 eh, el;
-                split16(o[4 * j + 2 * hh] * inv[hh], eh.x, el.x);
-                split16(o[4 * j + 2 * hh + 1] * inv[hh], eh.y, el.y);
-                *reinterpret_cast<__nv_bfloat162*>(p.cp_hi + e + 8 * j) = eh;
-                if (p.planes == 2) *reinterpret_cast<__nv_bfloat162*>(p.cp_lo + e + 8 * j) = el;
-              }
-            }
+          const int64_t o = (int64_t)row * N + n;
+          if (gi == 0) {
+            emit_store(e0, row, epilogue_value(a0, b0, 0, 0.f, 1.f, 0.f));
+            emit_store(e1, row, epilogue_value(a1, b1, 0, 0.f, 1.f, 0.f));
+          } else if (gi == 2) {
+            const float y0 = epilogue_value(a0, b0, B2A_ACT_GELU, 0.f, 1.f, 0.f), y1 = epilogue_value(a1, b1, B2A_ACT_GELU, 0.f, 1.f, 0.f);
+            __nv_bfloat162 h2, l2;
+            split16(y0, h2.x, l2.x);
+            split16(y1, h2.y, l2.y);
+            *reinterpret_cast<__nv_bfloat162*>(p.fp_hi + o) = h2;
+            if (p.planes == 2) *reinterpret_cast<__nv_bfloat162*>(p.fp_lo + o) = l2;
+          } else {
+            const float* res = gi == 1 ? p.h : p.t;
+            float* out = gi == 1 ? p.t : p.u;
+            const float2 r = *reinterpret_cast<const float2*>(res + o);
+            *reinterpret_cast<float2*>(out + o) = make_float2(epilogue_value(a0, b0, 0, 0.f, 1.f, r.x), epilogue_value(a1, b1, 0, 0.f, 1.f, r.y));
           }
         }
       }
-    } else {
-      const int which = stage == 3 ? 0 : 1;
-      const float* x = which ? p.u : p.t;
-      float* y = which ? p.h : p.t;
-      __nv_bfloat16* eh = which ? p.hp_hi : p.ap_hi;
-      __nv_bfloat16* el = p.planes == 2 ? (which ? p.hp_lo : p.ap_lo) : nullptr;
-      for (int row = bid * 8 + warp; row < p.T; row += grid * 8) {
+    } else if (un.s == 3 || un.s == 6) {
+      const int which = un.s == 6, row = m0 + un.col * LN_ROWS + warp;
+      if (row < p.T) {
+        const float* x = which ? p.u : p.t;
+        float* y = which ? p.h : p.t;
+        __nv_bfloat16* eh = which ? p.hp_hi : p.ap_hi;
+        __nv_bfloat16* el = p.planes == 2 ? (which ? p.hp_lo : p.ap_lo) : nullptr;
         const int64_t o = (int64_t)row * p.hs;
         layernorm_row_vec<8>(x + o, nullptr, y + o, p.hs, p.ln_w[which], p.ln_b[which], nullptr, p.eps, 0, 0, 0.f, eh + o,
                              el ? el + o : nullptr, lane);
       }
-    }
-    if constexpr (TL) { if (ct == 0) p.tl[((int64_t)k * grid + bid) * 2 + 1] = globaltimer(); }
-    if (k + 1 < total) {
-      fence_proxy_async_global();
-      bar_sync(1, 256);
-      if (ct == 0) { __threadfence(); grid_arrive(p.bar); }
+    } else {
+      float o[32], m[2] = {-INFINITY, -INFINITY}, lsum[2] = {0.f, 0.f};
+#pragma unroll
+      for (int j = 0; j < 32; j++) o[j] = 0.f;
+      const int kmax[2] = {p.T - 1, p.T - 1}, kmin[2] = {0, 0};
+      const uint64_t dqh = gmma_desc_sw128(sb + OFF_Q), dql = gmma_desc_sw128(sb + OFF_Q + PLANE);
+      mbar_wait(q_full, qn & 1);
+      for (int t = 0; t < p.nkt; t++, g++) {
+        const int s = g % SLOTS;
+        const uint32_t st = sb + s * SLOT_BYTES;
+        mbar_wait(full + s, (g / SLOTS) & 1);
+        if (wg == 0)
+          attn_tc_tile(o, m, lsum, dqh, dql, gmma_desc_sw128(st), gmma_desc_sw128(st + PLANE), gmma_desc_sw128(st + 2 * PLANE),
+                       gmma_desc_sw128(st + 3 * PLANE), t * 64, kmax, kmin, lane);
+        if ((ct & 127) == 0) mbar_arrive(empty + s);
+      }
+      if ((ct & 127) == 0) mbar_arrive(q_empty);
+      qn++;
+      if (wg == 0) {
+        const Unit ua = unit_of(p, opaque(G));
+        const int m0 = ua.m * 64;
+        float inv[2];
+        attn_tc_row_inv(lsum, inv);
+#pragma unroll
+        for (int hh = 0; hh < 2; hh++) {
+          const int q = m0 + w4 * 16 + (lane >> 2) + 8 * hh;
+          if (q < p.T) {
+            const int64_t e = (int64_t)q * p.hs + ua.col * 64 + 2 * (lane & 3);
+#pragma unroll
+            for (int j = 0; j < 8; j++) {
+              __nv_bfloat162 eh, el;
+              split16(o[4 * j + 2 * hh] * inv[hh], eh.x, el.x);
+              split16(o[4 * j + 2 * hh + 1] * inv[hh], eh.y, el.y);
+              *reinterpret_cast<__nv_bfloat162*>(p.cp_hi + e + 8 * j) = eh;
+              if (p.planes == 2) *reinterpret_cast<__nv_bfloat162*>(p.cp_lo + e + 8 * j) = el;
+            }
+          }
+        }
+      }
+    }
+    fence_proxy_async_global();
+    bar_sync(1, 256);
+    if (ct == 0) {
+      const Unit un2 = unit_of(p, opaque(G));
+      __threadfence();
+      arrive(arrival_of(p, un2.s, un2.m));
+    }
+    if constexpr (TL) {
+      if (ct == 0) {
+        const Unit un2 = unit_of(p, opaque(G));
+        p.tl[((int64_t)(un2.l * STAGES + un2.s) * gridDim.x + blockIdx.x) * 3 + 1] = globaltimer();
+      }
     }
   }
 }
@@ -317,7 +387,7 @@
 WsLayout ws_layout(int64_t T, int64_t H, int64_t hs, int64_t inter) {
   auto up = [](int64_t x) { return (x + 255) / 256 * 256; };
   WsLayout w;
-  int64_t o = 256;
+  int64_t o = CNT_BYTES;
   w.t = o; o += up(T * hs * 4);
   w.u = o; o += up(T * hs * 4);
   w.cp_hi = o; o += up(T * hs * 2);
@@ -326,7 +396,7 @@
   w.ap_lo = o; o += up(T * hs * 2);
   w.fp_hi = o; o += up(T * inter * 2);
   w.fp_lo = o; o += up(T * inter * 2);
-  w.attn = o; o += b2a_attention_tc_ws_bytes(1, (int32_t)H, (int32_t)T, (int32_t)T);
+  w.attn = o; o += b2a_attention_tc_ws_bytes(2, (int32_t)H, (int32_t)T, (int32_t)T);
   w.total = o;
   return w;
 }
@@ -335,13 +405,34 @@
 
 extern "C" int64_t b2a_albert_ws_bytes(int32_t T, int32_t heads, int32_t hidden, int32_t inter) {
   return ws_layout(T, heads, hidden, inter).total;
+}
+
+extern "C" int32_t b2a_albert_ws_regions(int32_t T, int32_t heads, int32_t hidden, int32_t inter, int64_t* out) {
+  const WsLayout L = ws_layout(T, heads, hidden, inter);
+  const int64_t H = heads, a = (int64_t)T * hidden * 4, b = (int64_t)T * hidden * 2, f = (int64_t)T * inter * 2;
+  int n = 0;
+  auto put = [&](int64_t off, int64_t bytes) { out[1 + 2 * n] = off; out[2 + 2 * n] = bytes; n++; };
+  out[0] = CNT_BYTES;
+  put(0, (MAX_MB + C_N * MAX_MB) * 4);
+  put(L.t, a); put(L.u, a); put(L.cp_hi, b); put(L.cp_lo, b); put(L.ap_hi, b); put(L.ap_lo, b); put(L.fp_hi, f); put(L.fp_lo, f);
+  const AttnOperands at = attn_operands((void*)(uintptr_t)L.attn, 2 * H, T, T);
+  const int64_t qk = H * T * 64, v = H * 64 * at.tkp;
+  for (int par = 0; par < 2; par++) {
+    const __half* pl[6] = {at.qh, at.ql, at.kh, at.kl, at.vh, at.vl};
+    for (int i = 0; i < 6; i++) {
+      const int64_t e = i < 4 ? qk : v;
+      put((int64_t)(uintptr_t)(pl[i] + par * e), e * 2);
+    }
+  }
+  return n;
 }
 
 extern "C" int32_t b2a_albert_encoder(const b2a_albert_t* a, void* ws, uint32_t* err, int64_t* timeline, void* stream) {
   B2A_CHECK_ARG(a && ws && err && a->h && a->h_hi && (a->planes == 1 || (a->planes == 2 && a->h_lo)), "null pointer");
   for (int i = 0; i < 4; i++) B2A_CHECK_ARG(a->w[i] && a->bias[i], "null weight or bias");
   for (int i = 0; i < 2; i++) B2A_CHECK_ARG(a->ln_w[i] && a->ln_b[i], "null LayerNorm parameter");
-  B2A_CHECK_ARG(a->T >= 64 && a->T <= 512 && a->layers > 0 && a->heads > 0 && a->hidden == 64 * a->heads && a->hidden <= 1024 &&
+  B2A_CHECK_ARG(a->grid >= 0, "grid: 0 (one CTA per SM) or a CTA count");
+  B2A_CHECK_ARG(a->T >= 64 && a->T <= 64 * MAX_MB && a->layers > 0 && a->heads > 0 && a->hidden == 64 * a->heads && a->hidden <= 1024 &&
                 a->inter % 64 == 0 && a->inter > 0, "shape: 64 <= T <= 512, hidden = 64 * heads <= 1024, inter a multiple of 64");
   const int T = a->T, H = a->heads, hs = a->hidden, inter = a->inter;
   uint8_t* base = (uint8_t*)ws;
@@ -361,8 +452,8 @@
   p.cp_hi = (__nv_bfloat16*)(base + L.cp_hi); p.cp_lo = (__nv_bfloat16*)(base + L.cp_lo);
   p.ap_hi = (__nv_bfloat16*)(base + L.ap_hi); p.ap_lo = (__nv_bfloat16*)(base + L.ap_lo);
   p.fp_hi = (__nv_bfloat16*)(base + L.fp_hi); p.fp_lo = (__nv_bfloat16*)(base + L.fp_lo);
-  p.attn = attn_operands(base + L.attn, H, T, T);
-  p.bar = (unsigned*)base; p.err = err;
+  p.attn = attn_operands(base + L.attn, 2 * H, T, T);
+  p.cnt = (unsigned*)base; p.err = err;
   p.tl = (long long*)timeline;
 
   AlbertMaps m;
@@ -376,8 +467,8 @@
     if (!e) e = map16(&m.a_lo[i], a->planes == 2 ? a_lo[i] : a_hi[i], 2, ad, as, false);
     if (!e) e = map16(&m.w[i], a->w[i], 2, wd, as, false);
   }
-  const uint64_t qd[3] = {64, (uint64_t)T, (uint64_t)H}, qs[2] = {128, (uint64_t)T * 128};
-  const uint64_t vd[3] = {(uint64_t)p.attn.tkp, 64, (uint64_t)H}, vs[2] = {(uint64_t)p.attn.tkp * 2, (uint64_t)p.attn.tkp * 128};
+  const uint64_t qd[3] = {64, (uint64_t)T, 2 * (uint64_t)H}, qs[2] = {128, (uint64_t)T * 128};
+  const uint64_t vd[3] = {(uint64_t)p.attn.tkp, 64, 2 * (uint64_t)H}, vs[2] = {(uint64_t)p.attn.tkp * 2, (uint64_t)p.attn.tkp * 128};
   if (!e) e = map16(&m.qh, p.attn.qh, 3, qd, qs, true);
   if (!e) e = map16(&m.ql, p.attn.ql, 3, qd, qs, true);
   if (!e) e = map16(&m.kh, p.attn.kh, 3, qd, qs, true);
@@ -402,9 +493,20 @@
     b2a_set_error("b2a_albert_encoder: the kernel cannot be resident (%s)", cudaGetErrorString(cudaGetLastError()));
     return B2A_E_CUDA;
   }
-  if (cudaMemsetAsync(p.bar, 0, 4, st) != cudaSuccess) { b2a_set_error("b2a_albert_encoder: %s", cudaGetErrorString(cudaGetLastError())); return B2A_E_CUDA; }
+  B2A_CHECK_ARG(a->grid <= nsm * per_sm, "grid: more CTAs than can be co-resident");
+  const int ncol[STAGES] = {3 * hs / 64, H, hs / 64, 64 / LN_ROWS, inter / 64, hs / 64, 64 / LN_ROWS};
+  p.ustart[0] = 0;
+  const int grid = a->grid ? a->grid : nsm;
+  p.ng = p.mb < grid ? p.mb : grid;
+  for (int s = 0; s < STAGES; s++) { p.ncol[s] = ncol[s]; p.ustart[s + 1] = p.ustart[s] + ncol[s]; }
+  p.ulayer = p.ustart[STAGES];
+  if (cudaMemsetAsync(p.cnt, 0, CNT_BYTES, st) != cudaSuccess) { b2a_set_error("b2a_albert_encoder: %s", cudaGetErrorString(cudaGetLastError())); return B2A_E_CUDA; }
+  if (timeline && cudaMemsetAsync(timeline, 0, (size_t)a->layers * STAGES * grid * 3 * sizeof(int64_t), st) != cudaSuccess) {
+    b2a_set_error("b2a_albert_encoder: %s", cudaGetErrorString(cudaGetLastError()));
+    return B2A_E_CUDA;
+  }
   cudaLaunchConfig_t cfg = {};
-  cfg.gridDim = dim3(nsm); cfg.blockDim = dim3(THREADS); cfg.dynamicSmemBytes = SMEM_BYTES; cfg.stream = st;
+  cfg.gridDim = dim3(grid); cfg.blockDim = dim3(THREADS); cfg.dynamicSmemBytes = SMEM_BYTES; cfg.stream = st;
   cudaLaunchAttribute at[1];
   at[0].id = cudaLaunchAttributeCooperative;
   at[0].val.cooperative = 1;
diff --git a/mlx_audio_b200/ops.py b/mlx_audio_b200/ops.py
--- a/mlx_audio_b200/ops.py
+++ b/mlx_audio_b200/ops.py
@@ -786,7 +786,7 @@
 
 
 def albert_encoder(h: torch.Tensor, hp: Planes, layers: int, qkv: ConvW, attn_out: ConvW, ffn: ConvW, ffn_out: ConvW, ln_attn, ln_full,
-                   *, heads: int, scale: float, eps: float, timeline: Optional[torch.Tensor] = None) -> None:
+                   *, heads: int, scale: float, eps: float, timeline: Optional[torch.Tensor] = None, grid: int = 0) -> None:
     if h.dtype != torch.float32 or not h.is_contiguous() or h.dim() != 3 or h.shape[0] != 1:
         raise ValueError(f"albert_encoder: h must be a contiguous float32 [1, T, hidden] tensor, got {tuple(h.shape)} {h.dtype}")
     T, hs = h.shape[1], h.shape[2]
@@ -805,6 +805,7 @@
     a.ln_w[1], a.ln_b[1] = ln_full[0].data_ptr(), ln_full[1].data_ptr()
     a.eps, a.scale = eps, scale
     a.h, a.h_hi, a.h_lo = h.data_ptr(), hp.hi.data_ptr(), _p(hp.lo)
+    a.grid = grid
     err = albert_error_word(h.device)
     ws = torch.empty(_lib.lib().b2a_albert_ws_bytes(T, heads, hs, inter), device=h.device, dtype=torch.uint8)
     _call("albert", _lib.lib().b2a_albert_encoder, 1, C.byref(a), ws.data_ptr(), err.data_ptr(), _p(timeline), _stream())
```
